# ShangtongZhang/DeepRL

Hardware: AMD Instinct MI355X
Metric: gradient-updates/sec (higher is better)
Workload: dtype f32; 1 GPU; DQN Breakout 84x84x4 uint8, NatureConvBody, batch 32, 1000000-frame HBM replay ring, centered RMSprop, clip 5 (BASELINE configs[1]); global_batch=32, parallelism=replicas x1, actor_in_step=True, async_actor=True, kernel_variant=530248191

## Files before the change

### deeprl_amd/csrc/actor_env.h

```cpp
#pragma once
#include "common.h"
#include <stddef.h>

constexpr int kMaxEnvSteps = 8;
constexpr size_t kPrmHeadBytes = offsetof(dra_dqn_step_params, idx);
constexpr int kAringSlots = 64;
constexpr size_t kAprmStride = 512;
static_assert(kPrmHeadBytes <= kAprmStride && kPrmHeadBytes % 4 == 0, "parameter ring entry");

__host__ __device__ __forceinline__ uint64_t mix64(uint64_t z) {
  z = (z ^ (z >> 30)) * 0xBF58476D1CE4E5B9ull;
  z = (z ^ (z >> 27)) * 0x94D049BB133111EBull;
  return z ^ (z >> 31);
}

__device__ __forceinline__ uint64_t synth_frame_word(uint64_t seed, int64_t counter, int64_t action, int w) {
  (void)action;
  return mix64(seed * 0x9E3779B97F4A7C15ull + (uint64_t)counter * 882ull + (uint64_t)w);
}
__device__ __forceinline__ double synth_reward(uint64_t seed, int64_t counter) {
  const uint64_t hh = mix64((seed + 1) * 0x9E3779B97F4A7C15ull + (uint64_t)counter);
  const uint32_t u = (uint32_t)(hh >> 32) % 10u;
  return (u == 0) ? -1.0 : ((u == 9) ? 1.0 : 0.0);
}
// ... 94 lines not shown
int dra_actor_c3fc4(const float* y2_planes, const float* w3, const float* b3, const float* w4, const float* b4, float* y3_planes,
                    float* h4, unsigned* flags, int* timeout_flag, void* stream);

typedef unsigned long long ll_t;

struct ActorPersistArgs {
  const float *w1, *b1, *w2, *b2, *w3, *b3, *w4, *b4, *wh, *bh;
  uint8_t* frames; uint8_t* actions; double* rewards; int32_t* masks;
  int64_t ring_cap;
  const uint8_t* aring; unsigned* seq;
  uint8_t* pend_frame; double* pend_reward; int32_t* pend_mask;
  float* q_out;
  float* h4_plain;
  ll_t *y1, *y2p, *y3p, *h4;
  int* abort_word;
  uint64_t seed;
  double coef;
  int done_period, n_actions, n_env;
  int* timeout_flag;
  const int* w4_valid;
  const unsigned long long* fs_count;
  const unsigned long long* fs_need;
  unsigned long long* fs_done_host;
};

constexpr size_t kPersistY1 = 32 * 400, kPersistY2 = 2 * 64 * 81, kPersistY3 = 2 * 64 * 49, kPersistH4 = 2 * 512;
constexpr size_t kPersistLLWords = kPersistY1 + kPersistY2 + kPersistY3 + kPersistH4;
constexpr int kPersistWgs = 32;
int dra_actor_persist(const ActorPersistArgs* a, void* stream);

constexpr int kChainPad = 32;
constexpr int kFwdChainCounters = 2 * DRA_MAX_Z * 32 * kChainPad;
void dra_conv_chain_attach_announce(unsigned long long* count);
void dra_conv_chain_attach_zero(unsigned* word);
int dra_conv_fwd_chain(const void* frames, const int64_t* idx, int64_t* idx_copy, const int64_t* idx_tagged,
                       const unsigned long long* update_seq, const int64_t* newest_off, int nz, const float* const* w1,
                       const float* const* b1, float* const* y1, const float* const* w2, const float* const* b2, float* const* y2,
                       const float* const* w3, const float* const* b3, float* const* y3, int batch, double u8_coef,
                       unsigned* done_counters, const unsigned* epoch, int* timeout_flag, const DraFc4Rider* rider,
                       unsigned* rider_count, int* rider_pending, int* rider_valid, void* stream);

void dra_conv_fwd_chain_level(unsigned epoch, unsigned* image, unsigned* arrivals);

int dra_bwd_chain_counters(void);
struct DraBwdChainFc {
  const float *dq, *h4, *dh4, *x3, *w4;
  float *dwh, *dbh, *dw4, *db4;
  int n_actions, in_features;
  double* sq_partials;
  int* n_sq_partials;
  const int64_t* head_action;
  int head_group;
};
int dra_conv_bwd_chain(const float* dy3, const float* y2, const float* wt3, float* dw3, float* db3, int64_t stride3, float* dy2,
                       const float* y1, const float* wt2, float* dw2, float* db2, int64_t stride2, float* dy1, const void* frames,
                       const int64_t* idx, float* dw1, float* db1, int64_t stride1, int batch, double u8_coef, int act,
                       const dra_fold_seg* fold3, const dra_fold_seg* fold2, float* grad, double* partials3, int* n_partials3,
                       double* partials2, int* n_partials2, double* reset_slots, int n_reset, unsigned* counters,
                       const unsigned* epoch, int* timeout_flag, const DraBwdChainFc* fc, void* stream);
int dra_bwd_chain_level(int batch, int fc_in_features, unsigned epoch, unsigned* image, unsigned* arrivals);
```

### deeprl_amd/csrc/fused.hip

```cpp
#include "oneshot_lin.h"
#include "dgrad_scatter.h"
#include "actor_env.h"
#include "per_chain2.h"
#include <stdlib.h>
#include <type_traits>

static int g_tuning = 511 | 4096 | 8192 | 16384 | 32768 | 131072 | 524288 | 1048576 | 8388608 | 16777216 | 33554432 | 67108864 | 134217728 | 268435456;

DRA_API int dra_set_tuning(int mask) {
  if (mask < 0) return DRA_EINVAL;
  g_tuning = mask;
  return DRA_OK;
}
DRA_API int dra_get_tuning(int* mask) {
  if (!mask) return DRA_EINVAL;
  static bool env_read = false;
  if (!env_read) {
    env_read = true;
    const char* e = getenv("DRA_TUNING");
    if (e && atoi(e) >= 0) g_tuning = atoi(e);
  }
  *mask = g_tuning;
  return DRA_OK;
}
// ... 251 lines not shown
static FoldRole make_fold_role(const dra_fold_seg* fold, float* grad, double* partials, double* reset_slots, int n_reset) {
  FoldRole f;
  f.grad = grad; f.slabs = fold->slabs; f.begin4 = fold->begin >> 2; f.count4 = fold->count >> 2;
  f.stride4 = fold->slab_stride >> 2; f.n_slabs = fold->n_slabs; f.partials = partials;
  f.reset_slots = reset_slots; f.n_reset = reset_slots ? n_reset : 0;
  return f;
}
static bool fold_ok(const dra_fold_seg* fold, const float* grad, const double* partials) {
  return fold && grad && partials && fold->slabs && fold->n_slabs >= 1 && fold->n_slabs <= FoldRole::NG * FoldRole::SPT &&
         fold->count >= 4 && !(fold->begin & 3) &&
         !(fold->count & 3) && !(fold->slab_stride & 3) && !((((uintptr_t)fold->slabs) | ((uintptr_t)grad)) & 15);
}

int dra_conv_bwd_fused_fold(int layer, const float* dy, const void* x, const float* wt, const float* xact, float* dw, float* db,
                            int64_t slab_stride, float* dx, int batch, int act, int variant, const dra_fold_seg* fold,
                            float* grad, double* fold_partials, int* n_fold_partials, double* reset_slots, int n_reset,
                            void* stream) {
  if (!dy || !x || !wt || !dx || !dw || !db || batch < 1 || !n_fold_partials || !fold_ok(fold, grad, fold_partials)) return DRA_EINVAL;
  if (!(variant & DRA_VAR_ONESHOT_WGRAD) || !(variant & DRA_VAR_ONESHOT_DGRAD)) return DRA_EINVAL;
  hipStream_t st = dra_stream(stream);
  const FoldRole f = make_fold_role(fold, grad, fold_partials, reset_slots, n_reset);
  *n_fold_partials = f.blocks();
  if (layer == 2)
    return conv_bwd_fused_t<G2, WG2l, WG2l, FoldRole>(dy, x, wt, xact, dw, db, slab_stride, 1, dx, batch, act, variant, st, f, f.blocks());
  if (layer == 3)
    return conv_bwd_fused_t<G3, WG3l, WG3l, FoldRole>(dy, x, wt, xact, dw, db, slab_stride, 1, dx, batch, act, variant, st, f, f.blocks());
  return DRA_EINVAL;
}

int dra_conv1_wgrad_fold(const float* dy, const void* x, const int64_t* idx, float* dw_slabs, float* db_slabs, int64_t slab_stride,
                         int batch, double u8_coef, int variant, const dra_fold_seg* fold, float* grad, double* fold_partials,
                         int* n_fold_partials, double* reset_slots, int n_reset, const PerChain2Args* chain, void* stream) {
  if (!dy || !x || !dw_slabs || !db_slabs || batch < 1 || !(variant & DRA_VAR_ONESHOT_WGRAD) || !n_fold_partials ||
      !fold_ok(fold, grad, fold_partials))
    return DRA_EINVAL;
  const FoldRole f = make_fold_role(fold, grad, fold_partials, reset_slots, n_reset);
  *n_fold_partials = f.blocks();
  if (chain) {
    if (chain->nb > 256) return DRA_EINVAL;
    ChainRole<2> cr;
    cr.a = *chain;
    auto rw = make_wgrad_one<WG1u>(dy, x, dw_slabs, db_slabs, slab_stride, batch, u8_coef);
    rw.sample_idx = idx;
    return launch_multi(rw, rw.blocks(), f, f.blocks(), cr, 1, dra_stream(stream));
  }
  NoRole none;
  auto rw = make_wgrad_one<WG1u>(dy, x, dw_slabs, db_slabs, slab_stride, batch, u8_coef);
  rw.sample_idx = idx;
  return launch_multi(rw, rw.blocks(), f, f.blocks(), none, 0, dra_stream(stream));
}

static bool fc_wgrad_one(int batch) { return batch <= 32; }
constexpr int kFcWgradNI = 8;
struct BwdChainN { int fd, fw, fh, d3, w3, d2, w2, w1, f3, f2; };
using BD3 = ConvDgradLin<G3, 1>;
using BD2 = ConvDgradLin<G2, 2>;
using FCD = LinDgradOne<512>;
using FCW = LinWgradOne<8>;
template <bool FC>
__global__ void __launch_bounds__(256) __attribute__((amdgpu_waves_per_eu(1, 2)))
bwd_chain_kernel(const FCD fd, const FCW fw, const HeadWgradRole fh, const BD3 d3, const WG3l w3, const BD2 d2, const WG2l w2,
                 const WG1u w1, const FoldRole f3, const FoldRole f2, const BwdChainN n) {
  extern __shared__ __attribute__((aligned(16))) float dyn_lds[];
  int b = blockIdx.x, first = 0;
  if constexpr (FC) {
    if (b < n.fd) { fd.run_<true>(b, dyn_lds); return; }
    b -= n.fd; first += n.fd;
    if (b < n.fw) { fw.run(b, dyn_lds, first); return; }
    b -= n.fw; first += n.fw;
    if (b < n.fh) { fh.run(b, dyn_lds, first); return; }
    b -= n.fh; first += n.fh;
  }
  if (b < n.d3) { d3.run_<FC, true>(b, dyn_lds, first); return; }
  b -= n.d3; first += n.d3;
  if (b < n.w3) { w3.run_<FC, true>(b, dyn_lds, first); return; }
  b -= n.w3; first += n.w3;
  if (b < n.d2) { d2.run_<true, true>(b, dyn_lds, first); return; }
  b -= n.d2; first += n.d2;
  if (b < n.w2) { w2.run_<true, true>(b, dyn_lds, first); return; }
  b -= n.w2; first += n.w2;
  if (b < n.w1) { w1.run_<true>(b, dyn_lds, first); return; }
  b -= n.w1;
  if (b < n.f3) { f3.run_<true>(b, dyn_lds); return; }
  b -= n.f3;
  f2.run_<true>(b, dyn_lds);
}

constexpr int kBwdChainCounters = (2 * 32 + 3) * kChainLine;
int dra_bwd_chain_counters(void) { return kBwdChainCounters; }
constexpr int kBwdChainA = 0, kBwdChainB = 32 * kChainLine, kBwdChainW3 = 64 * kChainLine, kBwdChainW2 = 65 * kChainLine,
              kBwdChainF = 66 * kChainLine;
struct BwdChainArrivals { unsigned d3, d2, w3, w2, fd; };
static int fc_dgrad_tiles(int in_features) { return (in_features + 31) / 32; }
static BwdChainArrivals bwd_chain_arrivals(int batch, int fc_in_features) {
  WG3l w3; w3.B = batch;
  WG2l w2; w2.B = batch;
  BwdChainArrivals n;
  n.d3 = BD3::WGS_PER_SAMPLE; n.d2 = BD2::WGS_PER_SAMPLE; n.w3 = (unsigned)w3.blocks(); n.w2 = (unsigned)w2.blocks();
  n.fd = fc_in_features > 0 ? (unsigned)(fc_dgrad_tiles(fc_in_features) * ((batch + 31) / 32)) : 0u;
  return n;
}
int dra_bwd_chain_level(int batch, int fc_in_features, unsigned epoch, unsigned* image, unsigned* arrivals) {
  if (batch < 1 || batch > 32 || !arrivals) return DRA_EINVAL;
  const BwdChainArrivals n = bwd_chain_arrivals(batch, fc_in_features);
  arrivals[0] = n.d3; arrivals[1] = n.d2; arrivals[2] = n.w3; arrivals[3] = n.w2; arrivals[4] = n.fd;
  if (!image) return DRA_OK;
  for (int i = 0; i < 32 * kChainLine; ++i) { image[kBwdChainA + i] = epoch * n.d3; image[kBwdChainB + i] = epoch * n.d2; }
  for (int i = 0; i < kChainLine; ++i) {
    image[kBwdChainW3 + i] = epoch * n.w3; image[kBwdChainW2 + i] = epoch * n.w2; image[kBwdChainF + i] = epoch * n.fd;
  }
  return DRA_OK;
}

int dra_conv_bwd_chain(const float* dy3, const float* y2, const float* wt3, float* dw3, float* db3, int64_t stride3, float* dy2,
                       const float* y1, const float* wt2, float* dw2, float* db2, int64_t stride2, float* dy1, const void* frames,
                       const int64_t* idx, float* dw1, float* db1, int64_t stride1, int batch, double u8_coef, int act,
                       const dra_fold_seg* fold3, const dra_fold_seg* fold2, float* grad, double* partials3, int* n_partials3,
                       double* partials2, int* n_partials2, double* reset_slots, int n_reset, unsigned* counters,
                       const unsigned* epoch, int* timeout_flag, const DraBwdChainFc* fc, void* stream) {
  if (!dy3 || !y2 || !wt3 || !dw3 || !db3 || !dy2 || !y1 || !wt2 || !dw2 || !db2 || !dy1 || !frames || !dw1 || !db1 || batch < 1 ||
      batch > 32 || !n_partials3 || !n_partials2 || !fold_ok(fold3, grad, partials3) || !fold_ok(fold2, grad, partials2) || !counters ||
      !epoch || !timeout_flag)
    return DRA_EINVAL;
  if (kWideLd4 && ((int64_t)fold3->n_slabs * fold3->slab_stride * 4 >= (1ll << 31) || (int64_t)fold2->n_slabs * fold2->slab_stride * 4 >= (1ll << 31)))
    return DRA_EINVAL;
  BD3 d3 = make_dgrad_one<G3, 1>(dy3, wt3, y2, dy2, batch, act);
  WG3l w3 = make_wgrad_one<WG3l>(dy3, y2, dw3, db3, stride3, batch, 1.0);
  BD2 d2 = make_dgrad_one<G2, 2>(dy2, wt2, y1, dy1, batch, act);
  WG2l w2 = make_wgrad_one<WG2l>(dy2, y1, dw2, db2, stride2, batch, 1.0);
  WG1u w1 = make_wgrad_one<WG1u>(dy1, frames, dw1, db1, stride1, batch, u8_coef);
  w1.sample_idx = idx;
  FoldRole f3 = make_fold_role(fold3, grad, partials3, nullptr, 0);
  FoldRole f2 = make_fold_role(fold2, grad, partials2, reset_slots, n_reset);
  BwdChainN n;
  n.fd = n.fw = n.fh = 0;
  n.d3 = d3.blocks(); n.w3 = w3.blocks(); n.d2 = d2.blocks(); n.w2 = w2.blocks(); n.w1 = w1.blocks(); n.f3 = f3.blocks(); n.f2 = f2.blocks();
  *n_partials3 = n.f3; *n_partials2 = n.f2;
  unsigned *cA = counters + kBwdChainA, *cB = counters + kBwdChainB, *cW3 = counters + kBwdChainW3, *cW2 = counters + kBwdChainW2,
           *cF = counters + kBwdChainF;
  const BwdChainArrivals na = bwd_chain_arrivals(batch, fc ? fc->in_features : 0);
  if (n.w3 != (int)na.w3 || n.w2 != (int)na.w2 || n.d3 != (int)na.d3 * batch || n.d2 != (int)na.d2 * batch) return DRA_EINVAL;
  ChainHook base;
  base.epoch = epoch; base.epoch_bias = 0; base.timeout_flag = timeout_flag;
  FCD fd = {};
  FCW fw = {};
  HeadWgradRole fh;
  fh.dq = nullptr; fh.h4 = nullptr; fh.dwh = nullptr; fh.dbh = nullptr; fh.B = 0; fh.A = 0;
  if (fc) {
    if (!fc->dq || !fc->h4 || !fc->dh4 || !fc->x3 || !fc->w4 || !fc->dwh || !fc->dbh || !fc->dw4 || !fc->db4 || fc->n_actions < 1 ||
        fc->in_features != G3::OC * G3::P || !fc->sq_partials || !fc->n_sq_partials || !fc_wgrad_one(batch))
      return DRA_EINVAL;
    fd.dy = fc->dh4; fd.w = fc->w4; fd.xact = fc->x3; fd.dx = const_cast<float*>(dy3); fd.B = batch; fd.I = fc->in_features; fd.act = act;
    fd.tiles_n = fc_dgrad_tiles(fc->in_features);
    fd.hook = base; fd.hook.done = cF;
    fw.dy = fc->dh4; fw.x = fc->x3; fw.dw = fc->dw4; fw.db = fc->db4; fw.partials = fc->sq_partials; fw.B = batch; fw.O = 512;
    fw.I = fc->in_features; fw.tiles_o = 512 / 32; fw.groups_i = (fd.tiles_n + kFcWgradNI - 1) / kFcWgradNI;
    fh.dq = fc->dq; fh.h4 = fc->h4; fh.dwh = fc->dwh; fh.dbh = fc->dbh; fh.B = batch; fh.A = fc->n_actions;
    if (fc->head_action && fc->head_group > 1 && fc->n_actions % fc->head_group == 0) { fh.action = fc->head_action; fh.group = fc->head_group; }
    n.fd = (int)na.fd; n.fw = fw.blocks(); n.fh = 2 * fc->n_actions;
    fh.partials = fc->sq_partials + n.fw;
    *fc->n_sq_partials = n.fw + 2 * fc->n_actions;
  }
  d3.hook = base; d3.hook.done = cA; d3.hook.done_stride = kChainLine;
  w3.hook = base; w3.hook.done = cW3;
  if (fc) {
    d3.hook.wait = cF; d3.hook.wait_stride = 0; d3.hook.wait_target = na.fd; d3.hook.slow = 1;
    w3.hook.wait = cF; w3.hook.wait_stride = 0; w3.hook.wait_target = na.fd; w3.hook.slow = 1;
  }
  d2.hook = base; d2.hook.wait = cA; d2.hook.wait_stride = kChainLine; d2.hook.wait_target = na.d3;
  d2.hook.done = cB; d2.hook.done_stride = kChainLine;
  w2.hook = base; w2.hook.wait = cA; w2.hook.wait_stride = kChainLine; w2.hook.wait_target = na.d3; w2.hook.done = cW2;
  w1.hook = base; w1.hook.wait = cB; w1.hook.wait_stride = kChainLine; w1.hook.wait_target = na.d2;
  f3.hook = base; f3.hook.wait = cW3; f3.hook.wait_target = na.w3; f3.hook.slow = 1;
  f2.hook = base; f2.hook.wait = cW2; f2.hook.wait_target = na.w2; f2.hook.slow = 1;
  constexpr int fa = BD3::LDS_FLOATS > WG3l::LDS_FLOATS ? BD3::LDS_FLOATS : WG3l::LDS_FLOATS;
  constexpr int fb = BD2::LDS_FLOATS > WG2l::LDS_FLOATS ? BD2::LDS_FLOATS : WG2l::LDS_FLOATS;
  constexpr int fcl = WG1u::LDS_FLOATS > FoldRole::LDS_FLOATS ? WG1u::LDS_FLOATS : FoldRole::LDS_FLOATS;
  constexpr int fab = fa > fb ? fa : fb, fl = fab > fcl ? fab : fcl;
  constexpr size_t bytes = (size_t)fl * sizeof(float);
  static_assert(bytes <= 64 * 1024, "LDS per workgroup of the chained backward launch");
  const int grid = n.fd + n.fw + n.fh + n.d3 + n.w3 + n.d2 + n.w2 + n.w1 + n.f3 + n.f2;
  if (fc) {
    constexpr size_t bytes_fc = (size_t)(FCD::LDS_FLOATS > fl ? FCD::LDS_FLOATS : fl) * sizeof(float);
    static_assert(bytes_fc <= 80 * 1024, "two workgroups of the chained backward launch per CU");
    static DraLdsAttr lds_attr;
    if (bytes_fc > 64 * 1024)
      if (int rc = dra_grant_lds(lds_attr, reinterpret_cast<const void*>(&bwd_chain_kernel<true>), bytes_fc)) return rc;
    hipLaunchKernelGGL(bwd_chain_kernel<true>, dim3(grid), dim3(256), bytes_fc, dra_stream(stream), fd, fw, fh, d3, w3, d2, w2, w1, f3, f2, n);
  } else {
    hipLaunchKernelGGL(bwd_chain_kernel<false>, dim3(grid), dim3(256), bytes, dra_stream(stream), fd, fw, fh, d3, w3, d2, w2, w1, f3, f2, n);
  }
  DRA_LAUNCH_CHECK();
  return DRA_OK;
}

int dra_fc_bwd_fused_sq_partials(int batch, int n_actions, int in_features) {
  const int tiles_i = (in_features + 31) / 32;
  const int nw = fc_wgrad_one(batch) ? (512 / 32) * ((tiles_i + kFcWgradNI - 1) / kFcWgradNI) : (512 / 64) * ((in_features + 1 + 63) / 64);
  return nw + 2 * n_actions;
}

int dra_fc_bwd_fused_sq(const float* dq, const float* h4, const float* dh4, const float* x3, const float* w4, float* dwh,
                        float* dbh, float* dw4, float* db4, float* dx3, int batch, int n_actions, int in_features, int act,
                        int variant, double* sq_partials, int* n_sq_partials, const int64_t* head_action, int head_group,
                        void* stream) {
  if (!dq || !h4 || !dh4 || !x3 || !w4 || !dwh || !dbh || !dw4 || !db4 || !dx3 || batch < 1 || n_actions < 1 ||
      in_features < 1 || !sq_partials || !n_sq_partials || !(variant & DRA_VAR_ONESHOT_DGRAD))
    return DRA_EINVAL;
  hipStream_t st = dra_stream(stream);
  constexpr int O = 512;
  LinDgradOne<O> rd;
  rd.dy = dh4; rd.w = w4; rd.xact = x3; rd.dx = dx3; rd.B = batch; rd.I = in_features; rd.act = act;
  rd.tiles_n = (in_features + 31) / 32;
  HeadWgradRole rh;
  rh.dq = dq; rh.h4 = h4; rh.dwh = dwh; rh.dbh = dbh; rh.B = batch; rh.A = n_actions;
  if (head_action && head_group > 1 && n_actions % head_group == 0) { rh.action = head_action; rh.group = head_group; }
  if (fc_wgrad_one(batch)) {
    constexpr int NI = kFcWgradNI;
    LinWgradOne<NI> rl;
    rl.dy = dh4; rl.x = x3; rl.dw = dw4; rl.db = db4; rl.partials = sq_partials; rl.B = batch; rl.O = O; rl.I = in_features;
    rl.tiles_o = O / 32; rl.groups_i = (rd.tiles_n + NI - 1) / NI;
    const int nw = rl.blocks();
    rh.partials = sq_partials + nw;
    *n_sq_partials = nw + 2 * n_actions;
    return launch_multi(rd, rd.tiles_n * ((batch + 31) / 32), rl, nw, rh, 2 * n_actions, st);
  }
  LinWgradSq<64, 64, 32> pw;
  pw.M = O; pw.N = in_features + 1; pw.K = batch; pw.I = in_features; pw.dy = dh4; pw.x = x3; pw.dw = dw4; pw.db = db4;
  pw.partials = sq_partials;
  auto rw = make_igemm_role(pw, 1);
  const int nw = igemm_blocks(rw, 1);
  rh.partials = sq_partials + nw;
  *n_sq_partials = nw + 2 * n_actions;
  return launch_multi(rd, rd.tiles_n * ((batch + 31) / 32), rw, nw, rh, 2 * n_actions, st);
}

DRA_API int dra_fc_bwd_fused(const float* dq, const float* h4, const float* dh4, const float* x3, const float* w4,
                             float* dwh, float* dbh, float* dw4, float* db4, float* dx3, int batch, int n_actions,
                             int in_features, int act, int variant, void* stream) {
  if (!dq || !h4 || !dh4 || !x3 || !w4 || !dwh || !dbh || !dw4 || !db4 || !dx3 || batch < 1 || n_actions < 1 ||
      in_features < 1)
// ... 100 lines not shown
```

### deeprl_amd/csrc/learner.hip

```cpp
#include "oneshot_lin.h"
#include "actor_env.h"
#include "per_chain2.h"
#include "cached_graph.h"
#include <new>
#include <stddef.h>
#include <stdlib.h>
#include <string.h>
#include <vector>

enum { K_GATHER, K_CONV1_F, K_CONV2_F, K_CONV3_F, K_FC4_F, K_HEAD, K_HEAD_BW, K_FC4_BW, K_FC4_BX, K_CONV3_BW, K_CONV3_BX,
       K_CONV2_BW, K_CONV2_BX, K_CONV1_BW, K_NORM, K_STEP, K_COUNT };

static const char* kKernelNames[K_COUNT] = {
  "gather", "conv1_fwd", "conv2_fwd", "conv3_fwd", "fc4_fwd", "head_loss", "head_bwd_w", "fc4_bwd_w", "fc4_bwd_x",
  "conv3_bwd_w", "conv3_bwd_x", "conv2_bwd_w", "conv2_bwd_x", "conv1_bwd_w", "grad_norm", "rmsprop_step"};

enum { P_W1, P_B1, P_W2, P_B2, P_W3, P_B3, P_W4, P_B4, P_WH, P_BH, P_COUNT };

constexpr int kFc4Split = 8;
constexpr int kFc4SplitWide = 28;
constexpr int kFc4SplitMid = 14;
static int fc4_ks(const struct dra_dqn_learner* l);
constexpr int kAprmSlots = 16;

// ... 43 lines not shown
  int ag_prev_par;
  hipEvent_t* tr_ev;
  int tr_cap, tr_n;
  double host_wait_s, host_call_s;
  int64_t host_calls;
  struct { CachedGraph g; const float* params; int n_env; } g_actor[5];
  float* pa[4];
  hipEvent_t pa_reader[4];
  int pa_cur;
  bool pa_valid;
  float* ah4;
  uint8_t* qs_stage;
  float* q_stage;
  unsigned* q_seq_dev;
  unsigned q_seq_host;
  CachedGraph g_q;
  uint8_t* aprm_ring;
  unsigned* aprm_seq_dev;
  unsigned* fc4_ticket;
  uint64_t aprm_seq;
  uint8_t* aring_dev;
  uint8_t* aring_stage;
  unsigned* aring_seq;
  uint8_t* pend_frame;
  double* pend_reward;
  int32_t* pend_mask;
  uint64_t aring_pushed, aring_issued;
  bool aring_primed;
  CachedGraph g_aring[4];
  int g_aring_nenv[4];
  hipEvent_t aprm_ev[16];
  bool aprm_used[16];
  hipStream_t side;
  hipEvent_t ev_fork, ev_join[4];
  hipEvent_t ev_actor_done, ev_gather_done, ev_step_done;
  hipEvent_t last_done;
  bool actor_pending;
  int step_per;
  float step_beta;
  int64_t* idx_pin[4];
  CachedGraph g_rd[4], g_rd_per[4], g_rd_per_b[4];
  hipEvent_t ev_upd[4];
  bool upd_used[4];
  int rd_slot;
  int keep_minibatch;
  struct { hipEvent_t ev; int n; int64_t slots[8]; } arec[8];
  int arec_count;
  hipEvent_t actor_last = nullptr;
  hipEvent_t ev[K_COUNT + 1];
  bool profiling;
  int only_kernel;
  int only_chain;
  unsigned* hchain_dev;
  bool defer;
  float* defer_dev;
  bool defer_host;
  int defer_q;
  int rider_q;
  int64_t defer_begin, defer_count;
  hipEvent_t ev_flush;
  int* timeout_flag;
  int64_t* idx_tag_pin[4];
  int64_t* idx_tag_dev;
  unsigned long long* rd_seq_dev;
  uint64_t rd_issued;
  float* sp_stage;
  hipEvent_t sp_ev[8];
  bool sp_used[8];
  int sp_k;
  int64_t* ui_stage;
  hipEvent_t ui_ev[8];
  bool ui_used[8];
  int ui_k;
  CachedGraph g_qa[2];
  hipEvent_t ev_hq[2];
  int64_t hq_updates;
  bool hq_seeded;
  dra_sumtree* per_tree;
  double* per_stat;
  dra_per_chain2_io* per2_io[4];
  void* per2_dev;
  int64_t* per2_idx;
  const uint32_t* per2_words;
  int split_q;
  hipEvent_t split_opt_prev;
  bool split_seed, split_open;
  bool per2_active;
  bool per2_ride;
  bool per2_split;
  PerChain2Args per2_args;
  unsigned* fchain_dev;
  bool fchain;
  unsigned* bchain_dev;
  bool bchain;
  unsigned long long* all_dev;
  int actor_cus;
  unsigned* aflags;
  bool fs, fs_on;
  unsigned long long* fs_count;
  uint64_t fs_issued;
  unsigned long long* fs_host;
  bool fs_graph[4];
  bool fs_agraph[4];
  bool fs_persist_taken;
  bool fs_capturing;
  uint64_t fs_need_next;
// ... 88 lines not shown
       (cfg->head_kind == DRA_HEAD_CATEGORICAL && !(cfg->v_max > cfg->v_min))))
    return DRA_EINVAL;
  dra_dqn_learner* l = new (std::nothrow) dra_dqn_learner();
  if (!l) return DRA_ENOMEM;
  memset(l, 0, sizeof(*l));
  l->c = *cfg; l->ring = ring; l->p = params; l->pt = target; l->g = grad; l->s1 = state1; l->s2 = state2;
  l->rd_slot = -1;
  l->only_kernel = -1;
  if (cfg->head_kind == DRA_HEAD_QUANTILE) l->c.double_q = 0;
  const int B = cfg->batch, A = cfg->n_actions;
  const int nz = l->c.double_q ? 3 : 2;
  const int NO = cfg->head_kind == DRA_HEAD_VANILLA ? A : A * cfg->n_atoms;
  l->n_out = NO;
  int rc = 0;
  for (int g = 0; g < 2; ++g) {
    rc |= (int)hipMalloc(&l->state_[g], (size_t)B * 4 * 7056);
    rc |= (int)hipMalloc(&l->next_state_[g], (size_t)B * 4 * 7056);
    rc |= (int)hipMalloc(&l->action_[g], (size_t)B * 8);
    rc |= alloc_f(&l->reward_[g], B); rc |= alloc_f(&l->mask_[g], B);
  }
  rc |= (int)hipMalloc(&l->act_state, (size_t)4 * 7056);
  rc |= (int)hipMalloc(&l->idx, (size_t)B * 8);
  for (int z = 0; z < nz; ++z) {
    rc |= alloc_f(&l->y1[z], (int64_t)B * 32 * 400); rc |= alloc_f(&l->y2[z], (int64_t)B * 64 * 81);
    rc |= alloc_f(&l->y3[z], (int64_t)B * 64 * 49); rc |= alloc_f(&l->q[z], (int64_t)B * NO);
  }
  rc |= alloc_f(&l->h4, (int64_t)3 * B * 512);
  rc |= (int)hipMalloc(&l->opt_step, sizeof(int64_t));
  if (!rc) rc |= (int)hipMemset(l->opt_step, 0, sizeof(int64_t));
  if (cfg->head_kind != DRA_HEAD_VANILLA) {
    const int N = cfg->n_atoms;
    rc |= alloc_f(&l->atoms, N); rc |= alloc_f(&l->qr_ws, (int64_t)B * N); rc |= alloc_f(&l->alog, NO);
    if (!rc) {
      float host_atoms[1024];
      const double step = ((double)cfg->v_max - (double)cfg->v_min) / (double)(N - 1);
      for (int i = 0; i < N; ++i) host_atoms[i] = (float)((double)cfg->v_min + (double)i * step);
      host_atoms[N - 1] = cfg->v_max;
      rc |= (int)hipMemcpy(l->atoms, host_atoms, (size_t)N * sizeof(float), hipMemcpyHostToDevice);
    }
  }
  rc |= alloc_f(&l->ay1, 32 * 400); rc |= alloc_f(&l->ay2, 64 * 81); rc |= alloc_f(&l->ay3, 64 * 49);
  rc |= alloc_f(&l->aq, A);
  rc |= alloc_f(&l->ay2p, 2 * 64 * 81); rc |= alloc_f(&l->ay3p, 2 * 64 * 49);
  rc |= alloc_f(&l->dq, (int64_t)B * NO); rc |= alloc_f(&l->dh4, (int64_t)B * 512);
  rc |= alloc_f(&l->dy3, (int64_t)B * 64 * 49); rc |= alloc_f(&l->dy2, (int64_t)B * 64 * 81);
  rc |= alloc_f(&l->dy1, (int64_t)B * 32 * 400);
  rc |= alloc_f(&l->delta, (cfg->head_kind == DRA_HEAD_QUANTILE && cfg->n_atoms > B) ? cfg->n_atoms : B);
  rc |= alloc_f(&l->prio, B); rc |= alloc_f(&l->weights, B);
  rc |= alloc_f(&l->samp_prob, B + 1);
  l->slab_stride = cfg->conv_end;
  rc |= alloc_f(&l->slabs, (int64_t)cfg->ksplit * l->slab_stride);
  if (cfg->variant >= 0) l->variant = cfg->variant;
  else rc |= dra_get_tuning(&l->variant);
  if ((l->variant & DRA_VAR_RING_DIRECT) &&
      (!(l->variant & DRA_VAR_ONESHOT_WGRAD) || !(l->variant & DRA_VAR_GATHER_ON_UPDATE) || !(l->variant & DRA_VAR_PINNED_IDX)))
    l->variant &= ~DRA_VAR_RING_DIRECT;
  if (cfg->head_kind != DRA_HEAD_VANILLA) {
    l->variant |= DRA_VAR_ACTOR_V2;
    l->variant &= ~(DRA_VAR_ACTOR_V3 | DRA_VAR_ACTOR_FUSED_HEAD | DRA_VAR_GATHER_IN_GRAPH);
  }
  if (l->variant & DRA_VAR_ONESHOT_WGRAD) {
    const int wi[3] = {P_W1, P_W2, P_W3};
    const int64_t seg_end[3] = {cfg->offset[P_W2], cfg->offset[P_W3], cfg->conv_end};
    for (int k = 0; k < 3; ++k) {
      l->lstride[k] = seg_end[k] - cfg->offset[wi[k]];
      rc |= dra_conv_wgrad_slabs(k + 1, B, cfg->ksplit, l->variant, &l->lnslabs[k]);
      if (rc) break;
      rc |= alloc_f(&l->lslabs[k], (int64_t)l->lnslabs[k] * l->lstride[k]);
      if (!rc) rc |= (int)hipMemset(l->lslabs[k], 0, (size_t)l->lnslabs[k] * l->lstride[k] * sizeof(float));
    }
  }
  l->n_partials = 2 * dra_norm_partials();
  if ((l->variant & DRA_VAR_LATE_FOLD) && (l->variant & DRA_VAR_ONESHOT_WGRAD) && (l->variant & DRA_VAR_ONESHOT_DGRAD) &&
      (l->variant & DRA_VAR_FUSED_BWD) && !rc && cfg->offset[P_W1] == 0 && l->lnslabs[1] <= 32 && l->lnslabs[2] <= 32) {
    dra_fold_seg s0;
    memset(&s0, 0, sizeof(s0));
    s0.begin = 0; s0.count = l->lstride[0]; s0.slabs = l->lslabs[0]; s0.slab_stride = l->lstride[0]; s0.n_slabs = l->lnslabs[0];
    if (dra_clip_step_late_blocks(&s0, &l->late_nfold) == DRA_OK) {
      const int64_t np = dra_fc_bwd_fused_sq_partials(cfg->batch, NO, 3136) + (l->lstride[2] / 4 + 63) / 64 + (l->lstride[1] / 4 + 63) / 64 + l->late_nfold;
      l->late = np <= dra_norm_partials_max();
    }
  }
  rc |= alloc_f(&l->ah4, 512);
  l->rider_q = -1;
  l->defer_begin = cfg->offset[P_W4];
  l->defer_count = cfg->offset[P_B4] - cfg->offset[P_W4];
  {
    const int need = DRA_VAR_DEFER_FC4 | DRA_VAR_RING_DIRECT | DRA_VAR_GATHER_ON_UPDATE | DRA_VAR_ACTOR_PARAMS | DRA_VAR_ACTOR_RING |
                     DRA_VAR_ACTOR_FUSED_CONV1 | DRA_VAR_ACTOR_MEGA | DRA_VAR_ONESHOT_FWD;
    l->defer = (l->variant & need) == need && l->late && cfg->head_kind == DRA_HEAD_VANILLA && cfg->optimizer == DRA_OPT_RMSPROP &&
               !cfg->double_q && cfg->batch > 16 && cfg->batch < 128 &&
               (l->defer_begin & 3) == 0 && (l->defer_count & 3) == 0 && l->defer_count == (int64_t)512 * 3136 &&
               l->defer_begin >= l->lstride[0];
  }
  l->fchain = (l->variant & DRA_VAR_FWD_CHAIN) && (l->variant & DRA_VAR_RING_DIRECT) && cfg->head_kind == DRA_HEAD_VANILLA &&
              !cfg->double_q && cfg->batch > 16 && cfg->batch <= 32;
  l->bchain = (l->variant & DRA_VAR_BWD_CHAIN) && (l->variant & DRA_VAR_RING_DIRECT) && l->late && cfg->head_kind == DRA_HEAD_VANILLA &&
              !cfg->double_q && cfg->batch > 16 && cfg->batch <= 32;
  rc |= (int)hipMalloc(&l->bchain_dev, (size_t)dra_bwd_chain_counters() * sizeof(unsigned));
  if (!rc) rc |= (int)hipMemset(l->bchain_dev, 0, (size_t)dra_bwd_chain_counters() * sizeof(unsigned));
  rc |= (int)hipMalloc(&l->defer_dev, 8 * sizeof(float));
  if (!rc) {
    const int init[8] = {0, 0, 1, 1, 1, 1, 0, 0};
    rc |= (int)hipMemcpy(l->defer_dev, init, sizeof(init), hipMemcpyHostToDevice);
  }
  {
    const int need = DRA_VAR_FLAG_SYNC | DRA_VAR_RING_DIRECT | DRA_VAR_GATHER_ON_UPDATE | DRA_VAR_PIPE_GATHER | DRA_VAR_ACTOR_PARAMS |
                     DRA_VAR_ACTOR_RING | DRA_VAR_ACTOR_FUSED_CONV1 | DRA_VAR_ACTOR_MEGA | DRA_VAR_ACTOR_PERSIST;
    l->fs = (l->variant & need) == need && l->fchain && cfg->head_kind == DRA_HEAD_VANILLA &&
            !(l->variant & (DRA_VAR_GATHER_IN_GRAPH | DRA_VAR_ACTOR_V3));
  }
  rc |= (int)hipMalloc(&l->fs_count, 256);
  if (!rc) rc |= (int)hipMemset(l->fs_count, 0, 256);
  rc |= (int)hipHostMalloc(&l->fs_host, (size_t)(8 + kAringSlots) * sizeof(unsigned long long), hipHostMallocDefault);
  if (!rc) memset(l->fs_host, 0, (size_t)(8 + kAringSlots) * sizeof(unsigned long long));
  rc |= (int)hipEventCreateWithFlags(&l->ev_fs, hipEventDisableTiming);
  rc |= (int)hipMalloc(&l->aflags, (size_t)kMaxEnvSteps * 4 * sizeof(unsigned));
  rc |= (int)hipMalloc(&l->hchain_dev, 256);
  if (!rc) rc |= (int)hipMemset(l->hchain_dev, 0, 256);
  rc |= (int)hipMalloc(&l->fchain_dev, (size_t)(kFwdChainCounters + 2) * sizeof(unsigned));
  if (!rc) rc |= (int)hipMemset(l->fchain_dev, 0, (size_t)(kFwdChainCounters + 2) * sizeof(unsigned));
  l->ah = false;
  if ((l->variant & DRA_VAR_TARGET_AHEAD) && l->fs && (l->variant & DRA_VAR_LANE_EAGER) && l->bchain && !cfg->double_q && B <= 32 &&
      (l->variant & DRA_VAR_ONESHOT_FWD)) {
    for (int k = 0; k < 2; ++k) {
      rc |= alloc_f(&l->ah_y1[k], (int64_t)B * 32 * 400); rc |= alloc_f(&l->ah_y2[k], (int64_t)B * 64 * 81);
      rc |= alloc_f(&l->ah_y3[k], (int64_t)B * 64 * 49); rc |= alloc_f(&l->ah_slabs[k], (int64_t)kFc4SplitWide * B * 512);
      rc |= (int)hipMalloc(&l->ah_chain[k], (size_t)(kFwdChainCounters + 2) * sizeof(unsigned));
      if (!rc) rc |= (int)hipMemset(l->ah_chain[k], 0, (size_t)(kFwdChainCounters + 2) * sizeof(unsigned));
    }
    for (int k = 0; k < 8; ++k) rc |= (int)hipHostMalloc(&l->ah_idx_pin[k], 1024 * sizeof(int64_t), hipHostMallocDefault);
    rc |= (int)hipMalloc(&l->ah_idx_copy, 1024 * sizeof(int64_t));
    rc |= (int)hipMalloc(&l->ah_done, 256);
    if (!rc) rc |= (int)hipMemset(l->ah_done, 0, 256);
  }
  {
    const size_t words = kPersistLLWords + 1;
    rc |= (int)hipMalloc(&l->all_dev, words * sizeof(unsigned long long));
    if (!rc) rc |= (int)hipMemset(l->all_dev, 0, words * sizeof(unsigned long long));
  }
  if (!rc) rc |= (int)hipMemset(l->aflags, 0, (size_t)kMaxEnvSteps * 4 * sizeof(unsigned));
  if (l->variant & DRA_VAR_ACTOR_PARAMS) { rc |= alloc_f(&l->pa[0], cfg->n_params); rc |= alloc_f(&l->pa[1], cfg->n_params); }
  if ((l->variant & DRA_VAR_ACTOR_PARAMS) && (l->variant & DRA_VAR_GATHER_ON_UPDATE)) {
    rc |= alloc_f(&l->pa[2], cfg->n_params); rc |= alloc_f(&l->pa[3], cfg->n_params);
  }
  if (l->variant & DRA_VAR_ACTOR_V3) {
    rc |= (int)hipHostMalloc(&l->aprm_ring, kAprmSlots * kAprmStride, hipHostMallocDefault);
    rc |= (int)hipMalloc(&l->aprm_seq_dev, sizeof(unsigned));
    rc |= (int)hipMalloc(&l->fc4_ticket, sizeof(unsigned));
    if (!rc) rc |= (int)hipMemset(l->aprm_seq_dev, 0, sizeof(unsigned));
    if (!rc) rc |= (int)hipMemset(l->fc4_ticket, 0, sizeof(unsigned));
    for (int k = 0; k < kAprmSlots; ++k) rc |= (int)hipEventCreateWithFlags(&l->aprm_ev[k], hipEventDisableTiming);
  }
  if (l->variant & DRA_VAR_ACTOR_RING) {
    rc |= (int)hipMalloc(&l->aring_dev, kAringSlots * kAprmStride);
    rc |= (int)hipHostMalloc(&l->aring_stage, kAringSlots * kAprmStride, hipHostMallocDefault);
    rc |= (int)hipMalloc(&l->aring_seq, sizeof(unsigned));
    rc |= (int)hipMalloc(&l->pend_frame, 7056);
    rc |= (int)hipMalloc(&l->pend_reward, sizeof(double));
    rc |= (int)hipMalloc(&l->pend_mask, sizeof(int32_t));
    if (!rc) rc |= (int)hipMemset(l->aring_seq, 0, sizeof(unsigned));
    if (!rc) rc |= (int)hipMemset(l->aring_dev, 0, kAringSlots * kAprmStride);
  }
  rc |= alloc_f(&l->fc4_slabs, (int64_t)3 * kFc4SplitWide * B * 512);
  rc |= alloc_f(&l->afc4_slabs, (int64_t)kFc4Split * 512);
  l->lin_ws_floats = (int64_t)3 * 32 * B * 512;
  rc |= alloc_f(&l->lin_ws, l->lin_ws_floats);
  rc |= (int)hipMalloc(&l->partials, (size_t)dra_norm_partials_max() * sizeof(double));
  rc |= alloc_f(&l->loss, 1); rc |= alloc_f(&l->norm, 1);
  if (l->variant & DRA_VAR_IDX_PREFETCH) {
    if (!(l->variant & DRA_VAR_RING_DIRECT) || cfg->ring_capacity >= (1ll << 40)) l->variant &= ~DRA_VAR_IDX_PREFETCH;
  }
// ... 31 lines not shown
  rc |= (int)hipMemset(l->slabs, 0, (size_t)cfg->ksplit * l->slab_stride * sizeof(float));
  rc |= (int)hipMemset(l->partials, 0, (size_t)dra_norm_partials_max() * sizeof(double));
  rc |= (int)hipMemset(l->prm_dev, 0, sizeof(dra_dqn_step_params));
  for (int k = 0; k <= K_COUNT; ++k) rc |= (int)hipEventCreate(&l->ev[k]);
  for (int k = 0; k < 8; ++k) rc |= (int)hipEventCreateWithFlags(&l->stage_ev[k], hipEventDisableTiming);
  for (int k = 0; k < 2; ++k) rc |= (int)hipEventCreateWithFlags(&l->ev_hq[k], hipEventDisableTiming);
  rc |= (int)hipStreamCreateWithFlags(&l->side, hipStreamNonBlocking);
  rc |= (int)hipEventCreateWithFlags(&l->ev_fork, hipEventDisableTiming);
  for (int k = 0; k < 4; ++k) rc |= (int)hipEventCreateWithFlags(&l->ev_join[k], hipEventDisableTiming);
  rc |= (int)hipEventCreateWithFlags(&l->ev_actor_done, hipEventDisableTiming);
  rc |= (int)hipEventCreateWithFlags(&l->ev_loss, hipEventDisableTiming);
  rc |= (int)hipEventCreateWithFlags(&l->ev_gather_done, hipEventDisableTiming);
  rc |= (int)hipEventCreateWithFlags(&l->ev_step_done, hipEventDisableTiming);
  rc |= (int)hipEventCreateWithFlags(&l->ev_flush, hipEventDisableTiming);
  for (int g = 0; g < 2; ++g) {
    rc |= (int)hipEventCreateWithFlags(&l->ev_mb_ready[g], hipEventDisableTiming);
    rc |= (int)hipEventCreateWithFlags(&l->ev_mb_free[g], hipEventDisableTiming);
  }
  if (rc) { delete l; return rc; }
  *out = l;
  return DRA_OK;
}

DRA_API int dra_dqn_learner_destroy(dra_dqn_learner* l) {
  if (!l) return DRA_OK;
  (void)hipDeviceSynchronize();
  l->g_update.reset();
  l->g_update_per.reset();
  l->g_q.reset();
  for (auto& g : l->g_ag) g.reset();
  for (auto& g : l->g_qa) g.reset();
  for (auto& ga : l->g_actor) ga.g.reset();
  for (int k = 0; k < 4; ++k) {
    l->g_pipe[k].reset(); l->g_pipe_per[k].reset(); l->g_pipe_per_b[k].reset();
    l->g_rd[k].reset(); l->g_rd_per[k].reset(); l->g_rd_per_b[k].reset();
    l->g_aring[k].reset();
  }
  if (l->tr_ev) {
    for (int i = 0; i < l->tr_cap * 5; ++i) (void)hipEventDestroy(l->tr_ev[i]);
    delete[] l->tr_ev;
  }
  for (int g = 0; g < 2; ++g) {
    (void)hipEventDestroy(l->ev_mb_ready[g]); (void)hipEventDestroy(l->ev_mb_free[g]);
    void* mb[] = {l->state_[g], l->next_state_[g], l->action_[g], l->reward_[g], l->mask_[g]};
    for (void* b : mb) if (b) (void)hipFree(b);
  }
  for (int k = 0; k < 4; ++k) if (l->pa[k]) (void)hipFree(l->pa[k]);
  if (l->ah4) (void)hipFree(l->ah4);
  if (l->defer_dev) (void)hipFree(l->defer_dev);
  if (l->aflags) (void)hipFree(l->aflags);
  if (l->all_dev) (void)hipFree(l->all_dev);
  if (l->fchain_dev) (void)hipFree(l->fchain_dev);
  if (l->hchain_dev) (void)hipFree(l->hchain_dev);
  for (int k = 0; k < 2; ++k) {
    void* ab[] = {l->ah_y1[k], l->ah_y2[k], l->ah_y3[k], l->ah_slabs[k], l->ah_chain[k]};
    for (void* b : ab) if (b) (void)hipFree(b);
  }
  for (int k = 0; k < 8; ++k) if (l->ah_idx_pin[k]) (void)hipHostFree(l->ah_idx_pin[k]);
  if (l->ah_idx_copy) (void)hipFree(l->ah_idx_copy);
  if (l->ah_done) (void)hipFree(l->ah_done);
  if (l->bchain_dev) (void)hipFree(l->bchain_dev);
  if (l->fs_count) (void)hipFree(l->fs_count);
  if (l->fs_host) (void)hipHostFree(l->fs_host);
  if (l->ev_fs) (void)hipEventDestroy(l->ev_fs);
  if (l->aring_dev) {
    (void)hipFree(l->aring_dev); (void)hipHostFree(l->aring_stage); (void)hipFree(l->aring_seq);
    (void)hipFree(l->pend_frame); (void)hipFree(l->pend_reward); (void)hipFree(l->pend_mask);
  }
  if (l->aprm_ring) {
    (void)hipHostFree(l->aprm_ring); (void)hipFree(l->aprm_seq_dev); (void)hipFree(l->fc4_ticket);
    for (int k = 0; k < kAprmSlots; ++k) (void)hipEventDestroy(l->aprm_ev[k]);
  }
  void* bufs[] = {l->act_state, l->idx, l->h4, l->ay1, l->ay2,
                  l->ay3, l->aq, l->dq, l->dh4, l->dy3, l->dy2, l->dy1, l->delta, l->prio, l->weights, l->samp_prob,
                  l->slabs, l->fc4_slabs, l->afc4_slabs, l->lin_ws, l->partials, l->loss, l->norm, l->prm_dev};
  for (void* b : bufs) if (b) (void)hipFree(b);
  void* hb[] = {l->atoms, l->qr_ws, l->alog, l->opt_step, l->ay2p, l->ay3p};
  for (void* b : hb) if (b) (void)hipFree(b);
  for (int k = 0; k < 3; ++k) if (l->lslabs[k]) (void)hipFree(l->lslabs[k]);
  for (int z = 0; z < 3; ++z) {
    if (l->y1[z]) (void)hipFree(l->y1[z]);
    if (l->y2[z]) (void)hipFree(l->y2[z]);
    if (l->y3[z]) (void)hipFree(l->y3[z]);
    if (l->q[z]) (void)hipFree(l->q[z]);
  }
  (void)hipHostFree(l->prm_stage);
  (void)hipHostFree(l->idx_stage);
  for (int k = 0; k < 4; ++k) {
    if (l->idx_pin[k]) (void)hipHostFree(l->idx_pin[k]);
    (void)hipEventDestroy(l->ev_upd[k]);
  }
  for (int k = 0; k < 4; ++k) if (l->idx_tag_pin[k]) (void)hipHostFree(l->idx_tag_pin[k]);
  if (l->idx_tag_dev) (void)hipFree(l->idx_tag_dev);
  if (l->per2_dev) (void)hipFree(l->per2_dev);
  if (l->per2_idx) (void)hipFree(l->per2_idx);
  if (l->rd_seq_dev) (void)hipFree(l->rd_seq_dev);
  if (l->sp_stage) (void)hipHostFree(l->sp_stage);
  for (int k = 0; k < 8; ++k) if (l->sp_ev[k]) (void)hipEventDestroy(l->sp_ev[k]);
  if (l->ui_stage) (void)hipHostFree(l->ui_stage);
  for (int k = 0; k < 8; ++k) if (l->ui_ev[k]) (void)hipEventDestroy(l->ui_ev[k]);
  if (l->timeout_flag) (void)hipHostFree(l->timeout_flag);
  if (l->qs_stage) (void)hipHostFree(l->qs_stage);
  if (l->q_stage) (void)hipHostFree(l->q_stage);
  if (l->q_seq_dev) (void)hipFree(l->q_seq_dev);
  for (int k = 0; k < 2; ++k) {
    if (l->ev_hq[k]) (void)hipEventDestroy(l->ev_hq[k]);
// ... 374 lines not shown

template <int KS>
__global__ void __launch_bounds__(256)
head_fused_kernel(const float* __restrict__ slabs, int nz, int B, int A, const float* __restrict__ b4_on,
                  const float* __restrict__ b4_tg, const float* __restrict__ wh_on, const float* __restrict__ wh_tg,
                  const float* __restrict__ bh_on, const float* __restrict__ bh_tg, const int64_t* __restrict__ action,
                  const float* __restrict__ reward, const float* __restrict__ mask, float gamma_n, int double_q,
                  float* __restrict__ h4_out, float* __restrict__ q_on, float* __restrict__ q_tg, float* __restrict__ q_on2,
                  float* __restrict__ delta, float* __restrict__ dq, float* __restrict__ dh4, int64_t* __restrict__ opt_step,
                  const RingScalars rs, const float* __restrict__ per_w, const float* __restrict__ pf_w4) {
  __shared__ float s_h[3][512];
  __shared__ float s_q[3][64];
  const int b = blockIdx.x, tid = threadIdx.x;
  if (b >= B) {
    const int pcol = (b - B) * 32;
    float4 v[16];
#pragma unroll
    for (int qq = 0; qq < 16; ++qq) {
      const int e = tid + 256 * qq, row = e >> 3, c4 = e & 7;
      v[qq] = *reinterpret_cast<const float4*>(pf_w4 + (int64_t)row * 3136 + pcol + 4 * c4);
    }
#pragma unroll
    for (int qq = 0; qq < 16; ++qq) asm volatile("" :: "v"(v[qq].x), "v"(v[qq].y), "v"(v[qq].z), "v"(v[qq].w));
    return;
  }
  head_fused_body<KS, false>(slabs, nz, B, A, b4_on, b4_tg, wh_on, wh_tg, bh_on, bh_tg, action, reward, mask, gamma_n, double_q, h4_out, q_on, q_tg, q_on2, delta, dq, dh4, opt_step, rs, per_w, b, s_h, s_q, nullptr);
}

struct HeadArgs {
  const float* slabs; int nz, B, A;
  const float *b4_on, *b4_tg, *wh_on, *wh_tg, *bh_on, *bh_tg;
  const int64_t* action; const float *reward, *mask; float gamma_n; int double_q;
  float *h4_out, *q_on, *q_tg, *q_on2, *delta, *dq, *dh4; int64_t* opt_step;
  RingScalars rs; const float* per_w; unsigned* done;
};
template <int KS>
__global__ void __launch_bounds__(256) __attribute__((amdgpu_waves_per_eu(1, 2)))
head_fc_bwd_kernel(const HeadArgs ha, const LinDgradOne<512> rd, const LinWgradOne<8> rl, const HeadWgradRole rh, const int nd, const int nw) {
  extern __shared__ __attribute__((aligned(16))) float dyn_lds[];
  int b = blockIdx.x;
  if (b < ha.B) {
    float (*s_h)[512] = reinterpret_cast<float (*)[512]>(dyn_lds);
    float (*s_q)[64] = reinterpret_cast<float (*)[64]>(dyn_lds + 3 * 512);
    head_fused_body<KS, true>(ha.slabs, ha.nz, ha.B, ha.A, ha.b4_on, ha.b4_tg, ha.wh_on, ha.wh_tg, ha.bh_on, ha.bh_tg, ha.action, ha.reward,
                              ha.mask, ha.gamma_n, ha.double_q, ha.h4_out, ha.q_on, ha.q_tg, ha.q_on2, ha.delta, ha.dq, ha.dh4, ha.opt_step,
                              ha.rs, ha.per_w, b, s_h, s_q, ha.done);
    return;
  }
  b -= ha.B;
  if (b < nd) { rd.run_<false, true>(b, dyn_lds); return; }
  b -= nd;
  if (b < nw) { rl.run_<true>(b, dyn_lds); return; }
  rh.run_<true>(b - nw, dyn_lds);
}

__global__ void __launch_bounds__(64)
head_wgrad_kernel(const float* __restrict__ dq, const float* __restrict__ h4, int B, int A, float* __restrict__ dwh,
                  float* __restrict__ dbh) {
  const int a = blockIdx.x, k = blockIdx.y * 64 + threadIdx.x;
  float acc = 0.f, accb = 0.f;
  int b = 0;
  for (; b + 8 <= B; b += 8) {
    float d[8], h[8];
#pragma unroll
    for (int i = 0; i < 8; ++i) { d[i] = dq[(int64_t)(b + i) * A + a]; h[i] = h4[(int64_t)(b + i) * 512 + k]; }
#pragma unroll
    for (int i = 0; i < 8; ++i) { acc += d[i] * h[i]; accb += d[i]; }
  }
  for (; b < B; ++b) {
    const float d = dq[(int64_t)b * A + a];
    acc += d * h4[(int64_t)b * 512 + k];
    accb += d;
  }
  dwh[a * 512 + k] = acc;
  if (k == 0) dbh[a] = accb;
}

#define STEP(kid, expr)                                                        \
  do {                                                                         \
    if (l->only_kernel >= 0 && l->only_kernel != (kid)) break;                 \
    if (l->profiling) DRA_HIP(hipEventRecord(l->ev[kid], st));                 \
    int _rc = (expr);                                                          \
    if (_rc != DRA_OK) return _rc;                                             \
  } while (0)

static int launch_gather(dra_dqn_learner* l, hipStream_t st, const int64_t* idx = nullptr) {
  l->last_gb = l->gb;
  return dra_ring_gather(l->ring, idx ? idx : l->idx, l->c.batch, l->state_[l->gb], l->next_state_[l->gb], l->action_[l->gb], nullptr, nullptr,
                         l->reward_[l->gb], l->mask_[l->gb], (void*)st);
}

struct BodyFlags {
  dra_dqn_learner* const l;
  BodyFlags(dra_dqn_learner* l_, int gb, int rd_slot = -1, int rider_q = -1, bool fs_capturing = false, bool per2_active = false,
            int only_kernel = -1, int only_chain = 0) : l(l_) {
    l->gb = gb; l->rd_slot = rd_slot; l->rider_q = rider_q; l->fs_capturing = fs_capturing; l->per2_active = per2_active;
    l->only_kernel = only_kernel; l->only_chain = only_chain;
  }
  BodyFlags(const BodyFlags&) = delete;
  BodyFlags& operator=(const BodyFlags&) = delete;
  ~BodyFlags() {
    l->gb = 0; l->rd_slot = -1; l->rider_q = -1; l->fs_capturing = false;
    l->per2_active = l->per2_ride = l->per2_split = false;
    l->only_kernel = -1; l->only_chain = 0;
  }
};
// ... 180 lines not shown
  if (fc4_ks(l) == kFc4SplitWide)
    hipLaunchKernelGGL(fc4_reduce_kernel<kFc4SplitWide>, dim3(B, nz), dim3(256), 0, st, (const float*)l->fc4_slabs, B, P + o[P_B4],
                       T + o[P_B4], l->h4, l->opt_step, rs);
  else if (fc4_ks(l) == kFc4SplitMid)
    hipLaunchKernelGGL(fc4_reduce_kernel<kFc4SplitMid>, dim3(B, nz), dim3(256), 0, st, (const float*)l->fc4_slabs, B, P + o[P_B4],
                       T + o[P_B4], l->h4, l->opt_step, rs);
  else
    hipLaunchKernelGGL(fc4_reduce_kernel<kFc4Split>, dim3(B, nz), dim3(256), 0, st, (const float*)l->fc4_slabs, B, P + o[P_B4],
                       T + o[P_B4], l->h4, l->opt_step, rs);
  DRA_LAUNCH_CHECK();
  int rc = DRA_OK;
  {
    const float* hx[3] = {l->h4, l->h4 + (int64_t)B * 512, l->h4 + (int64_t)2 * B * 512};
    const float* hw[3] = {P + o[P_WH], T + o[P_WH], P + o[P_WH]};
    const float* hb[3] = {P + o[P_BH], T + o[P_BH], P + o[P_BH]};
    if ((rc = dra_head_fwd_one(nz, hx, hw, hb, l->q, B, NO, s))) return rc;
  }
  if (c.head_kind == DRA_HEAD_CATEGORICAL) {
    const float* weights = nullptr;
    if (per) {
      if (!l->per2_active &&
          (rc = dra_per_weights(nullptr, l->samp_prob, B, beta, c.replay_eps, c.replay_alpha, nullptr, l->weights, s))) return rc;
      weights = l->weights;
    }
    rc = dra_c51_loss(l->q[0], l->q[1], c.double_q ? l->q[2] : nullptr, l->action_[l->gb], 1, l->reward_[l->gb], l->mask_[l->gb],
                      B, A, N, c.gamma_n, c.v_min, c.v_max, l->atoms, l->delta, l->dq, weights, s);
    if (rc) return rc;
    if (per && !l->per2_active &&
        (rc = dra_per_weights(l->delta, l->samp_prob, B, beta, c.replay_eps, c.replay_alpha, l->prio, nullptr, s))) return rc;
  } else {
    if (per) return DRA_EINVAL;
    rc = dra_qr_loss(l->q[0], l->q[1], l->action_[l->gb], 1, l->reward_[l->gb], l->mask_[l->gb], B, A, N, c.gamma_n, l->qr_ws,
                     l->delta, l->loss, l->dq, s);
    if (rc) return rc;
  }
  hipLaunchKernelGGL(dist_head_dgrad_kernel, dim3(B, 4), dim3(256), 0, st, (const float*)l->dq, P + o[P_WH], (const float*)l->h4,
                     (const int64_t*)l->action_[l->gb], N, NO, l->dh4);
  DRA_LAUNCH_CHECK();
  return DRA_OK;
}

static int run_body(dra_dqn_learner* l, hipStream_t st, int per, float beta, int fork, int part = 0) {
  const dra_dqn_config& c = l->c;
  l->captured = true;
  const int B = c.batch, A = c.n_actions;
  const int nz = c.double_q ? 3 : 2;
  void* s = (void*)st;
  const float* P = l->p;
  const float* T = l->pt;
  const int64_t* o = c.offset;
  const bool rd = l->rd_slot >= 0;
  const bool bchain = l->bchain && rd && !l->profiling && l->only_kernel < 0 && part == 0 && !per && !(l->per2_active && l->per2_ride);
  bool head_chain = false;
  void *ring_frames = nullptr, *ring_actions = nullptr, *ring_rewards = nullptr, *ring_masks = nullptr;
  int ring_h = 4, ring_n = 1;
  double ring_discount = 1.0;
  if (rd) {
    int rc0 = dra_ring_pointers(l->ring, &ring_frames, &ring_actions, &ring_rewards, &ring_masks);
    if (!rc0) rc0 = dra_ring_shape(l->ring, &ring_h, &ring_n);
    if (!rc0) rc0 = dra_ring_discount(l->ring, &ring_discount);
    if (rc0) return rc0;
    if (ring_h != 4) return DRA_EINVAL;
  }
  if (part != 2 && l->only_chain != 2) {
  const void* x1[3] = {l->state_[l->gb], l->next_state_[l->gb], l->next_state_[l->gb]};
  const float* w1[3] = {P + o[P_W1], T + o[P_W1], P + o[P_W1]};
  const float* b1[3] = {P + o[P_B1], T + o[P_B1], P + o[P_B1]};
  bool chain = false;
  if (rd) {
    const int64_t off[3] = {0, ring_n, ring_n};
    const bool dev_idx = per && l->per2_dev;
    const bool pf = (l->variant & DRA_VAR_IDX_PREFETCH) && !dev_idx;
    chain = l->fchain && !l->profiling && l->only_kernel < 0 && nz == 2;
    if (!chain && l->rider_q >= 0 && l->only_kernel < 0) {
      const DraFc4Rider r = fc4_rider(l, l->pa[l->rider_q]);
      const int nb = fc4_rider_blocks(r.count4);
      dra_conv_attach_rider(&r, 0, (nb * kRiderConv1Pct) / 100, nullptr, nullptr);
    }
    if (chain) {
      const float* w2c[3] = {P + o[P_W2], T + o[P_W2], P + o[P_W2]};
      const float* b2c[3] = {P + o[P_B2], T + o[P_B2], P + o[P_B2]};
      const float* w3c[3] = {P + o[P_W3], T + o[P_W3], P + o[P_W3]};
      const float* b3c[3] = {P + o[P_B3], T + o[P_B3], P + o[P_B3]};
      const bool riding = l->rider_q >= 0;
      DraFc4Rider rdr;
      if (riding) rdr = fc4_rider(l, l->pa[l->rider_q]);
      if (l->fs_capturing) dra_conv_chain_attach_announce(l->fs_count);
      if ((l->variant & DRA_VAR_HEAD_CHAIN) && l->hchain_dev) dra_conv_chain_attach_zero(l->hchain_dev);
      int rcc = dra_conv_fwd_chain(ring_frames, dev_idx ? l->per2_idx + (size_t)l->rd_slot * 1024 : l->idx_pin[l->rd_slot], l->idx,
                                   pf ? l->idx_tag_dev + (size_t)l->rd_slot * 1024 : nullptr, pf ? l->rd_seq_dev : nullptr, off,
                                   l->ah_mode ? 1 : nz,
                                   w1, b1, l->y1, w2c, b2c, l->y2, w3c, b3c, l->y3, B, c.u8_coef, l->fchain_dev,
                                   l->fchain_dev + kFwdChainCounters, l->timeout_flag, riding ? &rdr : nullptr,
                                   l->fchain_dev + kFwdChainCounters + 1, defer_pending_word(l),
                                   defer_valid_word(l, l->rider_q >= 0 ? l->rider_q : 0), s);
      if (rcc) return rcc;
      if (l->only_chain == 1) return DRA_OK;
      if (l->ah_mode == 2)
        if (int rct = ah_target_launches(l, st, (int)(l->step_no & 1), l->idx_pin[l->rd_slot], false, 0)) return rct;
    } else
    STEP(K_CONV1_F, dra_conv1_fwd_koc_ringbatch(ring_frames, dev_idx ? l->per2_idx + (size_t)l->rd_slot * 1024 : l->idx_pin[l->rd_slot], l->idx,
                                                pf ? l->idx_tag_dev + (size_t)l->rd_slot * 1024 : nullptr, pf ? l->rd_seq_dev : nullptr,
                                                off, nz, w1, b1, l->y1, B, c.u8_coef, DRA_ACT_RELU, s));
  } else {
    STEP(K_CONV1_F, dra_conv_fwd_koc(1, nz, x1, w1, b1, l->y1, B, 1, c.u8_coef, DRA_ACT_RELU, s));
  }
  const void* x2[3] = {l->y1[0], l->y1[1], l->y1[2]};
  const float* w2[3] = {P + o[P_W2], T + o[P_W2], P + o[P_W2]};
  const float* b2[3] = {P + o[P_B2], T + o[P_B2], P + o[P_B2]};
  if (!chain && rd && l->rider_q >= 0 && l->only_kernel < 0) {
    const DraFc4Rider r = fc4_rider(l, l->pa[l->rider_q]);
    const int nb = fc4_rider_blocks(r.count4);
    dra_conv_attach_rider(&r, (nb * kRiderConv1Pct) / 100, nb - (nb * kRiderConv1Pct) / 100, nullptr, nullptr);
  }
  if (!chain)
  STEP(K_CONV2_F, dra_conv_fwd_koc(2, nz, x2, w2, b2, l->y2, B, 0, 1.0, DRA_ACT_RELU, s));
  const void* x3[3] = {l->y2[0], l->y2[1], l->y2[2]};
  const float* w3[3] = {P + o[P_W3], T + o[P_W3], P + o[P_W3]};
  const float* b3[3] = {P + o[P_B3], T + o[P_B3], P + o[P_B3]};
  const float* x4[3] = {l->y3[0], l->y3[1], l->y3[2]};
  const float* w4[3] = {P + o[P_W4], T + o[P_W4], P + o[P_W4]};
  const int ks4 = fc4_ks(l);
  if (!chain && rd && l->rider_q >= 0 && l->only_kernel < 0)
    dra_conv_attach_rider(nullptr, 0, 0, defer_pending_word(l), defer_valid_word(l, l->rider_q));
  if (chain) {
  } else if ((l->variant & DRA_VAR_ONESHOT_FWD) && ks4 == kFc4SplitMid && nz == 2 && B <= 32)
    STEP(K_CONV3_F, dra_conv3_fwd_koc_pf(nz, x3, w3, b3, l->y3, B, DRA_ACT_RELU, w4, nz, s));
  else
  STEP(K_CONV3_F, dra_conv_fwd_koc(3, nz, x3, w3, b3, l->y3, B, 0, 1.0, DRA_ACT_RELU, s));
  if (chain && l->ah_mode == 2) x4[1] = l->ah_y3[l->step_no & 1];
  if (l->variant & DRA_VAR_ONESHOT_FWD) STEP(K_FC4_F, dra_linear_fwd_slabs_one((chain && l->ah_mode == 1) ? 1 : nz, x4, w4, B, 3136, 512, ks4, l->fc4_slabs, s));
  else STEP(K_FC4_F, dra_linear_fwd_slabs(nz, x4, w4, B, 3136, 512, kFc4Split, l->fc4_slabs, s));
  if (l->profiling) DRA_HIP(hipEventRecord(l->ev[K_HEAD], st));
  RingScalars rs;
  memset(&rs, 0, sizeof(rs));
  if (rd) {
    rs.idx = l->idx; rs.actions = (const uint8_t*)ring_actions; rs.rewards = (const double*)ring_rewards;
    rs.masks = (const int32_t*)ring_masks; rs.n_step = ring_n; rs.discount = ring_discount;
    rs.out_action = l->action_[l->gb]; rs.out_reward = l->reward_[l->gb]; rs.out_mask = l->mask_[l->gb];
    if ((l->variant & DRA_VAR_IDX_PREFETCH) && l->only_kernel < 0) rs.seq = l->rd_seq_dev;
    if (chain || bchain) rs.chain_epoch = l->fchain_dev + kFwdChainCounters;
    if (chain && l->ah_mode == 1) {
      rs.z1_slabs = l->ah_slabs[l->step_no & 1]; rs.z1_done = l->ah_done; rs.z1_want = l->step_no + 1ull; rs.z1_timeout = l->timeout_flag;
    }
  }
  if (l->only_kernel >= 0 && l->only_kernel != K_HEAD) {
  } else if (c.head_kind != DRA_HEAD_VANILLA) {
    int rc = run_dist_head(l, st, per, beta, rs);
    if (rc) return rc;
  } else {
    const float* per_w = (per && l->per2_active) ? l->weights : nullptr;
    head_chain = (l->variant & DRA_VAR_HEAD_CHAIN) && chain && !per && ks4 == kFc4SplitMid && B <= 32 && nz == 2 && l->late && part == 0 &&
                 !(l->variant & DRA_VAR_BWD_CHAIN_FC) && (l->variant & DRA_VAR_ONESHOT_DGRAD) && l->hchain_dev && !l->profiling;
    const bool pf = (l->variant & DRA_VAR_ONESHOT_DGRAD) && B % 8 == 0 && B <= 32 && dra_xcd_order_enabled();
    const float* pf_w4 = pf ? P + o[P_W4] : nullptr;
    const int hb = B + (pf ? 3136 / 32 : 0);
    l->q_head_chain = head_chain ? 1 : 0; l->q_head_pf = (!head_chain && pf) ? 1 : 0; l->q_head_launches++;
    if (head_chain) {
      HeadArgs ha;
      ha.slabs = l->fc4_slabs; ha.nz = nz; ha.B = B; ha.A = A; ha.b4_on = P + o[P_B4]; ha.b4_tg = T + o[P_B4]; ha.wh_on = P + o[P_WH];
      ha.wh_tg = T + o[P_WH]; ha.bh_on = P + o[P_BH]; ha.bh_tg = T + o[P_BH]; ha.action = (const int64_t*)l->action_[l->gb];
      ha.reward = (const float*)l->reward_[l->gb]; ha.mask = (const float*)l->mask_[l->gb]; ha.gamma_n = c.gamma_n; ha.double_q = c.double_q;
      ha.h4_out = l->h4; ha.q_on = l->q[0]; ha.q_tg = l->q[1]; ha.q_on2 = l->q[2]; ha.delta = l->delta; ha.dq = l->dq; ha.dh4 = l->dh4;
      ha.opt_step = l->opt_step; ha.rs = rs; ha.per_w = nullptr; ha.done = l->hchain_dev;
      ChainHook hk;
      hk.wait = l->hchain_dev; hk.wait_target = (unsigned)B; hk.timeout_flag = l->timeout_flag;
      LinDgradOne<512> rd = {};
      rd.dy = l->dh4; rd.w = P + o[P_W4]; rd.xact = l->y3[0]; rd.dx = l->dy3; rd.B = B; rd.I = 3136; rd.act = DRA_ACT_RELU; rd.tiles_n = 3136 / 32;
      rd.hook = hk;
      LinWgradOne<8> rl = {};
      float* Gh = l->g;
      rl.dy = l->dh4; rl.x = l->y3[0]; rl.dw = Gh + o[P_W4]; rl.db = Gh + o[P_B4]; rl.partials = l->partials; rl.B = B; rl.O = 512; rl.I = 3136;
      rl.tiles_o = 512 / 32; rl.groups_i = (rd.tiles_n + 8 - 1) / 8;
      rl.hook = hk;
      HeadWgradRole rh;
      rh.dq = l->dq; rh.h4 = l->h4; rh.dwh = Gh + o[P_WH]; rh.dbh = Gh + o[P_BH]; rh.B = B; rh.A = A;
      const int nd = rd.tiles_n, nw = rl.blocks();
      rh.partials = l->partials + nw;
      rh.hook = hk;
      if (nw + 2 * A != dra_fc_bwd_fused_sq_partials(B, A, 3136)) return DRA_EINVAL;
      constexpr size_t hbytes = (size_t)LinDgradOne<512>::LDS_FLOATS * sizeof(float);
      static DraLdsAttr lds_attr;
      if (int rcl = dra_grant_lds(lds_attr, reinterpret_cast<const void*>(&head_fc_bwd_kernel<kFc4SplitMid>), hbytes)) return rcl;
      hipLaunchKernelGGL(head_fc_bwd_kernel<kFc4SplitMid>, dim3(B + nd + nw + 2 * A), dim3(256), hbytes, st, ha, rd, rl, rh, nd, nw);
    } else
    if (ks4 == kFc4SplitWide)
      hipLaunchKernelGGL(head_fused_kernel<kFc4SplitWide>, dim3(hb), dim3(256), 0, st, (const float*)l->fc4_slabs, nz, B, A,
                         P + o[P_B4], T + o[P_B4], P + o[P_WH], T + o[P_WH], P + o[P_BH], T + o[P_BH],
                         (const int64_t*)l->action_[l->gb], (const float*)l->reward_[l->gb], (const float*)l->mask_[l->gb], c.gamma_n,
                         c.double_q,
                         l->h4, l->q[0], l->q[1], l->q[2], l->delta, l->dq, l->dh4, l->opt_step, rs, per_w, pf_w4);
    else if (ks4 == kFc4SplitMid)
      hipLaunchKernelGGL(head_fused_kernel<kFc4SplitMid>, dim3(hb), dim3(256), 0, st, (const float*)l->fc4_slabs, nz, B, A,
                         P + o[P_B4], T + o[P_B4], P + o[P_WH], T + o[P_WH], P + o[P_BH], T + o[P_BH],
                         (const int64_t*)l->action_[l->gb], (const float*)l->reward_[l->gb], (const float*)l->mask_[l->gb], c.gamma_n,
                         c.double_q,
                         l->h4, l->q[0], l->q[1], l->q[2], l->delta, l->dq, l->dh4, l->opt_step, rs, per_w, pf_w4);
    else
      hipLaunchKernelGGL(head_fused_kernel<kFc4Split>, dim3(hb), dim3(256), 0, st, (const float*)l->fc4_slabs, nz, B, A,
                         P + o[P_B4], T + o[P_B4], P + o[P_WH], T + o[P_WH], P + o[P_BH], T + o[P_BH],
                         (const int64_t*)l->action_[l->gb], (const float*)l->reward_[l->gb], (const float*)l->mask_[l->gb], c.gamma_n,
                         c.double_q,
                         l->h4, l->q[0], l->q[1], l->q[2], l->delta, l->dq, l->dh4, l->opt_step, rs, per_w, pf_w4);
    DRA_LAUNCH_CHECK();
    if (per && !per_w) {
      int rc = dra_td_loss(l->q[0], l->q[1], c.double_q ? l->q[2] : nullptr, l->action_[l->gb], 1, l->reward_[l->gb],
                           l->mask_[l->gb], B, A, c.gamma_n,
                           l->samp_prob, beta, c.replay_eps, c.replay_alpha, l->loss, l->dq, l->delta, l->prio, l->weights, s);
      if (rc) return rc;
      rc = dra_linear_bwd_x(l->dq, P + o[P_WH], l->h4, l->dh4, B, 512, A, DRA_ACT_RELU, s);
      if (rc) return rc;
    }
  }
  }
  if (part == 1) return DRA_OK;
  const int NO = l->n_out;
  float* G = l->g;
  float* S = l->slabs;
  if (l->variant & (DRA_VAR_FUSED_BWD | DRA_VAR_ONESHOT_WGRAD)) {
    const int var = l->variant;
    const bool own = var & DRA_VAR_ONESHOT_WGRAD;
    float* dw[3]; float* dbs[3]; int64_t stride[3];
    const int wi[3] = {P_W1, P_W2, P_W3}, bi_[3] = {P_B1, P_B2, P_B3};
    for (int k = 0; k < 3; ++k) {
      dw[k] = own ? l->lslabs[k] : S + o[wi[k]];
      dbs[k] = own ? l->lslabs[k] + (o[bi_[k]] - o[wi[k]]) : S + o[bi_[k]];
      stride[k] = own ? l->lstride[k] : l->slab_stride;
    }
    if (l->profiling) { DRA_HIP(hipEventRecord(l->ev[K_HEAD_BW], st)); DRA_HIP(hipEventRecord(l->ev[K_FC4_BW], st)); }
    if (l->late) {
      dra_fold_seg segs[3];
      conv_fold_segs(l, segs);
      const int nfc_expect = dra_fc_bwd_fused_sq_partials(B, NO, 3136), n3_expect = (int)((l->lstride[2] / 4 + 63) / 64), n2_expect = (int)((l->lstride[1] / 4 + 63) / 64);
      const bool fc_in_chain = bchain && (l->variant & DRA_VAR_BWD_CHAIN_FC) && B <= 32 && !head_chain;
      int nfc = (l->only_kernel >= 0 || (l->only_chain == 2 && !fc_in_chain) || head_chain) ? nfc_expect : 0, n3 = l->only_kernel >= 0 ? n3_expect : 0, n2 = l->only_kernel >= 0 ? n2_expect : 0;
      if (l->only_chain != 2 && !fc_in_chain && !head_chain)
      STEP(K_FC4_BX, dra_fc_bwd_fused_sq(l->dq, l->h4, l->dh4, l->y3[0], P + o[P_W4], G + o[P_WH], G + o[P_BH], G + o[P_W4],
                                         G + o[P_B4], l->dy3, B, NO, 3136, DRA_ACT_RELU, var, l->partials, &nfc,
                                         c.head_kind != DRA_HEAD_VANILLA ? l->action_[l->gb] : nullptr, c.n_atoms, s));
      if (l->profiling) DRA_HIP(hipEventRecord(l->ev[K_CONV3_BW], st));
      if (bchain) {
        DraBwdChainFc fcb;
        if (fc_in_chain) {
          fcb.dq = l->dq; fcb.h4 = l->h4; fcb.dh4 = l->dh4; fcb.x3 = l->y3[0]; fcb.w4 = P + o[P_W4]; fcb.dwh = G + o[P_WH];
          fcb.dbh = G + o[P_BH]; fcb.dw4 = G + o[P_W4]; fcb.db4 = G + o[P_B4]; fcb.n_actions = NO; fcb.in_features = 3136;
          fcb.sq_partials = l->partials; fcb.n_sq_partials = &nfc;
          fcb.head_action = c.head_kind != DRA_HEAD_VANILLA ? l->action_[l->gb] : nullptr; fcb.head_group = c.n_atoms;
        }
        int rcb = dra_conv_bwd_chain(l->dy3, l->y2[0], P + o[P_W3], dw[2], dbs[2], stride[2], l->dy2, l->y1[0], P + o[P_W2], dw[1],
                                     dbs[1], stride[1], l->dy1, ring_frames, l->idx, dw[0], dbs[0], stride[0], B, c.u8_coef,
                                     DRA_ACT_RELU, &segs[2], &segs[1], G, l->partials + nfc_expect, &n3,
                                     l->partials + nfc_expect + n3_expect, &n2,
                                     l->partials + nfc_expect + n3_expect + n2_expect, l->late_nfold, l->bchain_dev,
                                     l->fchain_dev + kFwdChainCounters, l->timeout_flag, fc_in_chain ? &fcb : nullptr, s);
        if (rcb) return rcb;
        if (nfc != nfc_expect || n3 != n3_expect || n2 != n2_expect) return DRA_EINVAL;
        l->late_nprior = nfc + n3 + n2;
        return DRA_OK;
      }
      if (l->per2_active && l->per2_ride)
        STEP(K_CONV3_BX, dra_conv3_bwd_fused_chain(l->dy3, l->y2[0], P + o[P_W3], l->y2[0], dw[2], dbs[2], stride[2], l->dy2, B,
                                                   DRA_ACT_RELU, var, &l->per2_args, l->per2_split ? 1 : 0, s));
      else
      STEP(K_CONV3_BX, dra_conv_bwd_fused(3, l->dy3, l->y2[0], P + o[P_W3], l->y2[0], dw[2], dbs[2], stride[2], c.ksplit,
                                          l->dy2, B, 0, 1.0, DRA_ACT_RELU, var, s));
      if (l->profiling) DRA_HIP(hipEventRecord(l->ev[K_CONV2_BW], st));
      STEP(K_CONV2_BX, dra_conv_bwd_fused_fold(2, l->dy2, l->y1[0], P + o[P_W2], l->y1[0], dw[1], dbs[1], stride[1], l->dy1, B,
                                               DRA_ACT_RELU, var, &segs[2], G, l->partials + nfc, &n3, nullptr, 0, s));
      STEP(K_CONV1_BW, dra_conv1_wgrad_fold(l->dy1, rd ? ring_frames : (const void*)l->state_[l->gb], rd ? l->idx : nullptr, dw[0],
                                            dbs[0], stride[0], B, c.u8_coef, var, &segs[1], G, l->partials + nfc + n3, &n2,
                                            l->partials + nfc_expect + n3_expect + n2_expect, l->late_nfold,
                                            (l->per2_active && l->per2_ride && l->per2_split) ? &l->per2_args : nullptr, s));
      if (nfc != nfc_expect || n3 != n3_expect || n2 != n2_expect) return DRA_EINVAL;
      l->late_nprior = nfc + n3 + n2;
      if (l->profiling) { DRA_HIP(hipEventRecord(l->ev[K_NORM], st)); DRA_HIP(hipEventRecord(l->ev[K_STEP], st)); }
      return DRA_OK;
    }
    STEP(K_FC4_BX, dra_fc_bwd_fused(l->dq, l->h4, l->dh4, l->y3[0], P + o[P_W4], G + o[P_WH], G + o[P_BH], G + o[P_W4],
                                    G + o[P_B4], l->dy3, B, NO, 3136, DRA_ACT_RELU, var, s));
    if (l->profiling) DRA_HIP(hipEventRecord(l->ev[K_CONV3_BW], st));
    if (l->per2_active && l->per2_ride)
      STEP(K_CONV3_BX, dra_conv3_bwd_fused_chain(l->dy3, l->y2[0], P + o[P_W3], l->y2[0], dw[2], dbs[2], stride[2], l->dy2, B,
                                                 DRA_ACT_RELU, var, &l->per2_args, 0, s));
    else
    STEP(K_CONV3_BX, dra_conv_bwd_fused(3, l->dy3, l->y2[0], P + o[P_W3], l->y2[0], dw[2], dbs[2], stride[2], c.ksplit,
                                        l->dy2, B, 0, 1.0, DRA_ACT_RELU, var, s));
    if (l->profiling) DRA_HIP(hipEventRecord(l->ev[K_CONV2_BW], st));
    STEP(K_CONV2_BX, dra_conv_bwd_fused(2, l->dy2, l->y1[0], P + o[P_W2], l->y1[0], dw[1], dbs[1], stride[1], c.ksplit,
                                        l->dy1, B, 0, 1.0, DRA_ACT_RELU, var, s));
    if (rd) {
      STEP(K_CONV1_BW, dra_conv1_wgrad_ringbatch(l->dy1, ring_frames, l->idx, dw[0], dbs[0], stride[0], B, c.u8_coef, var, s));
    } else {
      STEP(K_CONV1_BW, dra_conv_bwd_fused(1, l->dy1, l->state_[l->gb], nullptr, nullptr, dw[0], dbs[0], stride[0], c.ksplit, nullptr,
                                          B, 1, c.u8_coef, DRA_ACT_RELU, var, s));
    }
    if (own) {
      dra_fold_seg segs[3];
      conv_fold_segs(l, segs);
      int np_out = 0;
      STEP(K_NORM, dra_grad_sqnorm_segs(G, c.n_params, segs, 3, l->partials, &np_out, s));
      l->n_partials = np_out;
      if (l->profiling) DRA_HIP(hipEventRecord(l->ev[K_STEP], st));
      return DRA_OK;
    }
    const int np = dra_norm_partials();
    STEP(K_NORM, dra_grad_sqnorm(G, c.conv_end, S, c.ksplit, l->slab_stride, l->partials, s));
    if (l->profiling) DRA_HIP(hipEventRecord(l->ev[K_STEP], st));
// ... 248 lines not shown
      for (int r = 0; r < reps && rcb == DRA_OK; ++r) {
        if (pass == 0) rcb = run_body(l, st, 0, 0.f, 0);
        else hipLaunchKernelGGL(empty_probe_kernel, dim3(224), dim3(256), 0, st, (const int*)nullptr);
      }
      return rcb;
    });
    if (rc == DRA_OK) rc = g.launch(st);
    if (rc == DRA_OK) rc = (int)hipStreamSynchronize(st);
    float best = 0.f;
    for (int t = 0; t < 3 && rc == DRA_OK; ++t) {
      float ms = 0.f;
      rc = timed_replay(g, st, l->ev[0], l->ev[1], &ms);
      if (t == 0 || ms < best) best = ms;
    }
    g.reset();
    if (rc != DRA_OK) return rc;
    us[pass] = best * 1e3f / (float)reps;
  }
  out_us[0] = us[0];
  out_us[1] = us[1];
  return DRA_OK;
}

DRA_API int dra_dqn_learner_chain_replay(dra_dqn_learner* l, int which, int reps, float* out_us, void* stream) {
  if (!l || !out_us || reps < 1 || reps > 4096 || which < 0 || which > 1) return DRA_EINVAL;
  if (!(l->variant & DRA_VAR_RING_DIRECT) || !l->late || (which == 0 ? !l->fchain : !l->bchain) || l->c.double_q) return DRA_EINVAL;
  if (int rcl = fs_leave_any(l)) return rcl;
  hipStream_t st = dra_stream(stream);
  if (int rcf = flush_fc4(l, st)) return rcf;
  DRA_HIP(hipStreamSynchronize(st));
  unsigned* epoch = l->fchain_dev + kFwdChainCounters;
  float us[2] = {0.f, 0.f};
  for (int pass = 0; pass < 2; ++pass) {
    CachedGraph g = {};
    int rc = g.capture(st, [&] {
      BodyFlags f(l, 0, 0, -1, false, false, -1, which + 1);
      int rcb = DRA_OK;
      for (int r = 0; r < reps && rcb == DRA_OK; ++r) {
        if (which == 1) hipLaunchKernelGGL(chain_epoch_bump_kernel, dim3(1), dim3(1), 0, st, epoch);
        if (pass == 0) rcb = run_body(l, st, 0, 0.f, 0);
        else hipLaunchKernelGGL(empty_probe_kernel, dim3(224), dim3(256), 0, st, (const int*)nullptr);
        if (which == 0) hipLaunchKernelGGL(chain_epoch_bump_kernel, dim3(1), dim3(1), 0, st, epoch);
      }
      return rcb;
    });
    float best = 0.f;
    for (int t = 0; t < 4 && rc == DRA_OK; ++t) {
      float ms = 0.f;
      rc = timed_replay(g, st, l->ev[0], l->ev[1], &ms);
      if (t == 1 || (t > 1 && ms < best)) best = ms;
    }
    if (rc == DRA_OK) rc = (int)hipMemsetAsync(l->fchain_dev, 0, (size_t)(kFwdChainCounters + 1) * sizeof(unsigned), st);
    if (rc == DRA_OK) rc = (int)hipMemsetAsync(l->bchain_dev, 0, (size_t)dra_bwd_chain_counters() * sizeof(unsigned), st);
    if (rc == DRA_OK) rc = (int)hipStreamSynchronize(st);
    g.reset();
    if (rc != DRA_OK) return rc;
    us[pass] = best * 1e3f / (float)reps;
  }
  out_us[0] = us[0];
  out_us[1] = us[1];
  return *l->timeout_flag ? DRA_ETIMEDOUT : DRA_OK;
}

DRA_API int dra_dqn_learner_chain_set_epoch(dra_dqn_learner* l, uint64_t epoch, int64_t* arrivals, int n_arrivals, void* stream) {
  if (!l || !arrivals || n_arrivals < 8 || epoch > 0xffffffffull) return DRA_EINVAL;
  if (!l->fchain && !l->bchain) return DRA_EINVAL;
  if (int rcl = fs_leave_any(l)) return rcl;
  hipStream_t st = dra_stream(stream);
  if (int rcf = flush_fc4(l, st)) return rcf;
  DRA_HIP(hipStreamSynchronize(st));
  if (l->ah_stream) DRA_HIP(hipStreamSynchronize(l->ah_stream));
  const unsigned e = (unsigned)epoch;
  for (int i = 0; i < 8; ++i) arrivals[i] = 0;
  unsigned fa[2] = {0, 0}, ba[5] = {0, 0, 0, 0, 0};
  std::vector<unsigned> img((size_t)kFwdChainCounters + 1);
  dra_conv_fwd_chain_level(e, img.data(), fa);
  img[kFwdChainCounters] = e;
  DRA_HIP(hipMemcpy(l->fchain_dev, img.data(), img.size() * sizeof(unsigned), hipMemcpyHostToDevice));
  if (l->fchain) { arrivals[0] = fa[0]; arrivals[1] = fa[1]; }
  for (int k = 0; k < 2; ++k)
    if (l->ah_chain[k]) {
      DRA_HIP(hipMemcpy(l->ah_chain[k], img.data(), img.size() * sizeof(unsigned), hipMemcpyHostToDevice));
      arrivals[7] = 1;
    }
  if (l->bchain) {
    const bool fc = (l->variant & DRA_VAR_BWD_CHAIN_FC) != 0;
    std::vector<unsigned> bimg((size_t)dra_bwd_chain_counters());
    if (int rcb = dra_bwd_chain_level(l->c.batch, fc ? 3136 : 0, e, bimg.data(), ba)) return rcb;
    DRA_HIP(hipMemcpy(l->bchain_dev, bimg.data(), bimg.size() * sizeof(unsigned), hipMemcpyHostToDevice));
    for (int i = 0; i < 5; ++i) arrivals[2 + i] = ba[i];
  }
  return DRA_OK;
}

DRA_API int dra_dqn_learner_last_minibatch(dra_dqn_learner* l, void** state, void** next_state, void** action, void** reward,
                                           void** mask) {
  if (!l) return DRA_EINVAL;
  const int g = l->last_gb;
  if (state) *state = l->state_[g];
  if (next_state) *next_state = l->next_state_[g];
  if (action) *action = l->action_[g];
  if (reward) *reward = l->reward_[g];
  if (mask) *mask = l->mask_[g];
  return DRA_OK;
}

DRA_API int dra_dqn_learner_invalidate_actor_copy(dra_dqn_learner* l) {
  if (!l) return DRA_EINVAL;
  l->pa_valid = false;
  l->hq_updates = 0;
  l->hq_seeded = false;
  return DRA_OK;
}

DRA_API int dra_dqn_learner_kernel_name(int k, char* out, int n) {
  if (k < 0 || k >= K_COUNT || !out || n < 1) return DRA_EINVAL;
  strncpy(out, kKernelNames[k], (size_t)n - 1);
  out[n - 1] = 0;
  return DRA_OK;
}

DRA_API int dra_dqn_learner_kernel_count(void) { return K_COUNT; }

DRA_API int dra_dqn_learner_sync_target(dra_dqn_learner* l, void* stream) {
  if (!l) return DRA_EINVAL;
  if (int rcf = flush_fc4(l, dra_stream(stream))) return rcf;
  return dra_copy_f32(l->pt, l->p, l->c.n_params, stream);
}

__global__ void __launch_bounds__(256)
env_stack_kernel(const dra_dqn_step_params* __restrict__ prm, int e, uint8_t* __restrict__ frames,
                 double* __restrict__ rewards, int32_t* __restrict__ masks, int64_t capacity, uint64_t seed,
                 int done_period, uint8_t* __restrict__ stack) {
  const int j = blockIdx.x;
  const int64_t newest = prm->slot[e];
  const int64_t counter = prm->counter[e];
  int64_t slot = newest - 3 + j;
  if (slot < 0) slot += capacity;
  uint64_t* dst = reinterpret_cast<uint64_t*>(stack + (int64_t)j * 7056);
  uint64_t* src = reinterpret_cast<uint64_t*>(frames + slot * 7056);
  if (j == 3 && counter >= 0) {
    const uint64_t base = seed * 0x9E3779B97F4A7C15ull + (uint64_t)counter * 882ull;
    for (int w = threadIdx.x; w < 882; w += blockDim.x) {
// ... 1073 lines not shown
  int rc;
  bool seeded = false;
  const int par = (int)(l->step_no & 1);
  if (prm->n_env > 0) {
    if (l->mb_used[par]) DRA_HIP(hipStreamWaitEvent(sa, l->ev_mb_free[par], 0));
    memcpy(l->prm_stage[k].idx, prm->idx, (size_t)B * sizeof(int64_t));
    DRA_HIP(hipMemcpyAsync(l->prm_dev, &l->prm_stage[k], kPrmHeadBytes + (size_t)B * sizeof(int64_t), hipMemcpyHostToDevice, sa));
    TRACE(0, sa);
    if (l->pa_valid && l->pa_cur != par) l->pa_valid = false;
    if (l->last_done) DRA_HIP(hipStreamWaitEvent(sa, l->last_done, 0));
    if (!l->pa_valid) {
      if ((rc = seed_actor_copy(l, sa, par))) return rc;
      seeded = true;
    }
    if ((rc = ag_graph(l, prm->n_env, par, sa))) return rc;
    DRA_HIP(hipEventRecord(l->ev_mb_ready[par], sa));
    DRA_HIP(hipEventRecord(l->ev_actor_done, sa));
    l->actor_pending = true;
    TRACE(1, sa);
    TRACE(2, sa);
  }
  DRA_HIP(hipEventRecord(l->stage_ev[k], sa));
  if (do_update && l->ag_have_prev) {
    const int q = l->ag_prev_par;
    DRA_HIP(hipStreamWaitEvent(su, l->ev_mb_ready[q], 0));
    if (seeded) DRA_HIP(hipStreamWaitEvent(su, l->ev_join[0], 0));
    TRACE(3, su);
    if ((rc = pipe_graph(l, su, q))) return rc;
    TRACE(4, su);
    if (l->tr_ev && l->tr_n < l->tr_cap) l->tr_n++;
    DRA_HIP(hipEventRecord(l->ev_mb_free[q], su));
    l->last_done = l->ev_mb_free[q];
    l->mb_used[q] = true;
    if (l->pa_valid) l->pa_cur = q;
    l->ag_have_prev = false;
  }
  if (prm->n_env > 0) {
    l->ag_have_prev = true;
    l->ag_prev_par = par;
    l->step_no++;
  }
  return DRA_OK;
}

__global__ void fs_bump_kernel(unsigned long long* count) { __hip_atomic_fetch_add(count, 1ull, __ATOMIC_RELAXED, __HIP_MEMORY_SCOPE_AGENT); }

static int fs_leave(dra_dqn_learner* l, hipStream_t su, hipStream_t sa);
static int fs_leave_any(dra_dqn_learner* l) { return l->fs_on ? fs_leave(l, l->fs_su, l->fs_sa) : DRA_OK; }
static int fs_leave(dra_dqn_learner* l, hipStream_t su, hipStream_t sa) {
  if (!l->fs_on) return DRA_OK;
  l->fs_on = false;
  DRA_HIP(hipStreamSynchronize(su));
  DRA_HIP(hipStreamSynchronize(sa));
  if (l->ah && l->ah_stream) {
    DRA_HIP(hipStreamSynchronize(l->ah_stream));
    l->ah_valid = false;
    l->ah_next_set = false;
    DRA_HIP(hipMemsetAsync(l->fchain_dev, 0, (size_t)(kFwdChainCounters + 1) * sizeof(unsigned), su));
    DRA_HIP(hipMemsetAsync(l->bchain_dev, 0, (size_t)dra_bwd_chain_counters() * sizeof(unsigned), su));
    DRA_HIP(hipStreamSynchronize(su));
  }
  l->last_done = nullptr;
  for (int q = 0; q < 4; ++q) { l->pa_reader[q] = nullptr; l->upd_used[q] = false; l->fs_reader[q] = 0; }
  for (int k = 0; k < 8; ++k) l->stage_used[k] = false;
  l->arec_count = 0;
  l->fs_arec_n = 0;
  DRA_HIP(hipEventRecord(l->ev_fs, sa));
  l->actor_last = l->ev_fs;
  return DRA_OK;
}

static inline uint64_t fs_actor_done(const dra_dqn_learner* l) { return __atomic_load_n(&l->fs_host[0], __ATOMIC_ACQUIRE); }

static inline bool fs_reached(uint64_t done32, uint64_t target) { return (uint32_t)((uint32_t)done32 - (uint32_t)target) < 0x80000000u; }

static int fs_wait_actor(dra_dqn_learner* l, uint64_t target) {
  if (fs_reached(fs_actor_done(l), target)) return DRA_OK;
  HostTimeScope waited(l->host_wait_s);
  for (;;) {
    for (int i = 0; i < 64; ++i) {
      if (fs_reached(fs_actor_done(l), target)) return DRA_OK;
      __builtin_ia32_pause();
    }
    if (*l->timeout_flag) return DRA_ETIMEDOUT;
    if (waited.seconds() > 20.0) return DRA_ETIMEDOUT;
  }
}

static bool fs_eligible(const dra_dqn_learner* l, const dra_dqn_step_params* prm, int do_update, void* stream_actor) {
  if (!l->fs || !stream_actor || !do_update || prm->n_env < 1 || l->step_per || l->keep_minibatch || l->tr_ev) return false;
  const int q = (int)(l->step_no & 3), qr = (q + 3) & 3;
  if (!l->pa_valid || l->pa_cur != qr) return false;
  if (!l->g_rd[q].ready || !l->fs_graph[q]) return false;
  if (!l->g_aring[qr].ready || !l->fs_agraph[qr] || l->g_aring_nenv[qr] != prm->n_env) return false;
  if (!l->aring_primed || l->aring_issued >= l->aring_pushed) return false;
  if (l->defer ? (l->defer_host && l->defer_q != qr) : l->defer_host) return false;
  return true;
}

static int rd_eager(dra_dqn_learner* l, hipStream_t st, int q) {
  l->gb = q & 1;
  l->rd_slot = q;
  l->rider_q = l->defer ? ((q + 3) & 3) : -1;
  l->fs_capturing = true;
  int rc = run_body(l, st, 0, 0.f, 0, 0);
  l->fs_capturing = false;
  l->rider_q = -1;
  if (rc == DRA_OK) rc = launch_optimizer(l, st, l->pa[q], l->defer ? q : -1);
  l->gb = 0;
  l->rd_slot = -1;
  if (rc != DRA_OK) return rc;
  l->fs_issued++;
  if (l->defer) { l->defer_host = true; l->defer_q = q; }
  return DRA_OK;
}

static int step_lane(dra_dqn_learner* l, const dra_dqn_step_params* prm, hipStream_t su, hipStream_t sa) {
  const int B = l->c.batch;
  const int q = (int)(l->step_no & 3), cur = (q + 3) & 3;
  int rc;
  if (!l->fs_on) {
    DRA_HIP(hipStreamSynchronize(su));
    DRA_HIP(hipStreamSynchronize(sa));
    __atomic_store_n(&l->fs_host[0], (unsigned long long)(uint32_t)l->aring_issued, __ATOMIC_RELEASE);
    for (int i = 0; i < 4; ++i) l->fs_reader[i] = 0;
    l->fs_arec_n = 0;
    l->fs_on = true;
    l->fs_stat[1]++;
  }
  const dra_dqn_step_params* ablk =
      reinterpret_cast<const dra_dqn_step_params*>(l->aring_stage + (size_t)(l->aring_issued % kAringSlots) * kAprmStride);
  using clk = std::chrono::steady_clock;
  auto ns = [](clk::time_point a, clk::time_point b) { return (int64_t)std::chrono::duration_cast<std::chrono::nanoseconds>(b - a).count(); };
  const auto tp0 = clk::now();
  if (l->fs_reader[q]) {
    if ((rc = fs_wait_actor(l, l->fs_reader[q]))) return rc;
    l->fs_reader[q] = 0;
  }
  for (int i = l->fs_arec_n - 1; i >= 0; --i) {
    const auto& r = l->fs_arec[i];
    if (fs_reached(fs_actor_done(l), r.done_at)) continue;
    if (gather_reads_slots(l, prm->idx, r.slots, r.n)) {
      {
        HostTimeScope waited(l->host_wait_s);
        DRA_HIP(hipStreamSynchronize(sa));
      }
      l->fs_stat[3]++;
      break;
    }
  }
  const bool hazard = gather_reads_slots(l, prm->idx, ablk->slot, prm->n_env);
  const auto tp1 = clk::now();
  memcpy(l->idx_pin[q], prm->idx, (size_t)B * sizeof(int64_t));
  if (l->variant & DRA_VAR_IDX_PREFETCH) {
    const uint64_t tag = ((l->rd_issued + 1ull) & 0xffffffull) << 40;
    volatile int64_t* dst = l->idx_tag_pin[q];
    for (int b = 0; b < B; ++b) dst[b] = (int64_t)((uint64_t)prm->idx[b] | tag);
    DRA_HIP(hipMemcpyAsync(l->idx_tag_dev + (size_t)q * 1024, l->idx_tag_pin[q], (size_t)B * sizeof(int64_t), hipMemcpyHostToDevice, l->side));
// ... 23 lines not shown
  if (!l->fs_on) return DRA_EINVAL;
  if (hazard) {
    hipLaunchKernelGGL(fs_bump_kernel, dim3(1), dim3(1), 0, su, l->fs_count);
    DRA_LAUNCH_CHECK();
    l->fs_issued++;
    l->fs_stat[2]++;
  }
  l->fs_need_next = l->fs_issued;
  const auto tp3 = clk::now();
  if ((rc = issue_actor_ring(l, prm->n_env, l->pa[cur], cur, sa, true))) return rc;
  const auto tp4 = clk::now();
  l->fs_stat[4] += ns(tp0, tp1); l->fs_stat[5] += ns(tp1, tp2); l->fs_stat[6] += ns(tp2, tp3); l->fs_stat[7] += ns(tp3, tp4);
  l->actor_pending = true;
  const uint64_t done_at = l->aring_issued;
  l->fs_reader[cur] = done_at;
  if (l->fs_arec_n == 4) { for (int i = 1; i < 4; ++i) l->fs_arec[i - 1] = l->fs_arec[i]; l->fs_arec_n = 3; }
  auto& r = l->fs_arec[l->fs_arec_n++];
  r.done_at = done_at; r.n = prm->n_env;
  for (int e = 0; e < prm->n_env && e < 8; ++e) r.slots[e] = ablk->slot[e];
  l->pa_cur = q;
  if (l->ah && l->ah_stream && l->ah_next_set) {
    l->ah_next_set = false;
    bool ok = l->aring_issued < l->aring_pushed;
    for (int i = 0; ok && i < l->fs_arec_n; ++i) {
      const auto& ar = l->fs_arec[i];
      if (!fs_reached(fs_actor_done(l), ar.done_at) && gather_reads_slots(l, l->ah_next_idx, ar.slots, ar.n)) ok = false;
    }
    if (ok) {
      const dra_dqn_step_params* nblk =
          reinterpret_cast<const dra_dqn_step_params*>(l->aring_stage + (size_t)(l->aring_issued % kAringSlots) * kAprmStride);
      if (gather_reads_slots(l, l->ah_next_idx, nblk->slot, nblk->n_env)) ok = false;
    }
    if (ok) {
      const uint64_t nxt = l->step_no + 1;
      int64_t* pin = l->ah_idx_pin[nxt & 7];
      memcpy(pin, l->ah_next_idx, (size_t)B * sizeof(int64_t));
      hipLaunchKernelGGL(ah_gate_kernel, dim3(1), dim3(1), 0, l->ah_stream, (const unsigned long long*)l->fs_count,
                         (unsigned long long)ah_need, l->timeout_flag);
      DRA_LAUNCH_CHECK();
      if ((rc = ah_target_launches(l, l->ah_stream, (int)(nxt & 1), pin, true, nxt + 1ull))) return rc;
      memcpy(l->ah_idx, l->ah_next_idx, (size_t)B * sizeof(int64_t));
      l->ah_for_step = nxt;
      l->ah_valid = true;
    } else {
      l->ah_stat[2]++;
    }
  }
  l->step_no++;
  l->fs_stat[0]++;
  l->fs_stat[8] += ns(tp0, clk::now());
  return DRA_OK;
}

DRA_API int dra_dqn_learner_set_ahead_stream(dra_dqn_learner* l, void* stream) {
  if (!l) return DRA_EINVAL;
  if (int rcl = fs_leave_any(l)) return rcl;
  if (!stream || !l->ah_done) { l->ah = false; l->ah_stream = nullptr; return DRA_OK; }
  l->ah_stream = dra_stream(stream);
  l->ah = true;
  return DRA_OK;
}

DRA_API int dra_dqn_learner_stage_next_indices(dra_dqn_learner* l, const int64_t* idx_next, int n) {
  if (!l || !idx_next || n != l->c.batch || n > 1024) return DRA_EINVAL;
  if (!l->ah) return DRA_OK;
  memcpy(l->ah_next_idx, idx_next, (size_t)n * sizeof(int64_t));
  l->ah_next_set = true;
  return DRA_OK;
}

DRA_API int dra_dqn_learner_ahead_stats(dra_dqn_learner* l, int64_t* out) {
  if (!l || !out) return DRA_EINVAL;
  for (int i = 0; i < 4; ++i) out[i] = l->ah_stat[i];
  out[4] = l->ah ? 1 : 0;
  return DRA_OK;
}

DRA_API int dra_dqn_learner_path_flags(dra_dqn_learner* l, int64_t* out) {
  if (!l || !out) return DRA_EINVAL;
  const int64_t v[12] = {l->late, l->defer, l->fchain, l->bchain, l->fs, l->ah, l->q_per2_ride, l->q_head_chain, l->q_head_pf,
                         l->q_head_launches, (int64_t)l->variant, (l->timeout_flag && *l->timeout_flag) ? 1 : 0};
  for (int i = 0; i < 12; ++i) out[i] = v[i];
  return DRA_OK;
}

DRA_API int dra_dqn_learner_lane_stats(dra_dqn_learner* l, int64_t* out) {
  if (!l || !out) return DRA_EINVAL;
  for (int i = 0; i < 12; ++i) out[i] = l->fs_stat[i];
  return DRA_OK;
}

static int stage_acquire(dra_dqn_learner* l, int* k_out) {
  const int k = l->stage_k;
  l->stage_k = (k + 1) % 8;
  if (l->stage_used[k]) {
    HostTimeScope waited(l->host_wait_s);
    DRA_HIP(hipEventSynchronize(l->stage_ev[k]));
    if ((l->variant & DRA_VAR_GATHER_ON_UPDATE) && l->stage_used[(k + 1) % 8]) DRA_HIP(hipEventSynchronize(l->stage_ev[(k + 1) % 8]));
  }
  l->stage_used[k] = true;
  *k_out = k;
  return DRA_OK;
}

DRA_API int dra_dqn_learner_act(dra_dqn_learner* l, const dra_dqn_step_params* prm, int use_graph, void* stream) {
  if (!l || !prm || prm->n_env < 1 || prm->n_env > kMaxEnvSteps) return DRA_EINVAL;
// ... 226 lines not shown
```

### deeprl_amd/csrc/oneshot.h

```cpp
#pragma once
#include "igemm.h"

__device__ __forceinline__ int mfma_row(int r, int h) { return (r & 3) + 8 * (r >> 2) + 4 * h; }

__device__ __forceinline__ f32x16 zero16() {
  f32x16 a;
#pragma unroll
  for (int r = 0; r < 16; ++r) a[r] = 0.f;
  return a;
}

__device__ __forceinline__ void reduce4(float* __restrict__ red, const f32x16& acc, int wave, int lane, float out[4]) {
#pragma unroll
  for (int r = 0; r < 16; ++r) red[(wave * 16 + r) * 64 + lane] = acc[r];
  __syncthreads();
#pragma unroll
  for (int q = 0; q < 4; ++q) {
    const int r = wave * 4 + q;
    out[q] = (red[(0 * 16 + r) * 64 + lane] + red[(1 * 16 + r) * 64 + lane]) +
             (red[(2 * 16 + r) * 64 + lane] + red[(3 * 16 + r) * 64 + lane]);
  }
}

struct NoRole {
// ... 187 lines not shown
        reinterpret_cast<float4*>(grad)[begin4 + i] = r;
        sq = r.x * r.x + r.y * r.y + r.z * r.z + r.w * r.w;
      }
    }
    const double d = wave_sum((double)sq);
    if (tid == 0) partials[bid] = d;
  }
};

template <int O>
struct LinDgradOne {
  static constexpr int KW = O / 4, NJ = KW / 2, LDA = O + 1, RA = 32 * O / 256;
  static constexpr int LDS_FLOATS = 32 * LDA > 4096 ? 32 * LDA : 4096;
  static_assert(O % 8 == 0 && (32 * O) % 256 == 0, "reduction split over 4 waves x 2 half-waves");
  const float* dy;
  const float* w;
  const float* xact;
  float* dx;
  int B, I, act, tiles_n;
  ChainHook hook;
  __device__ __forceinline__ void run(int bid, float* __restrict__ lds, int = 0) const { run_<false>(bid, lds); }
  template <bool COUT, bool CIN = false>
  __device__ __forceinline__ void run_(int bid, float* __restrict__ lds) const {
    const int tid = threadIdx.x, wave = tid >> 6, lane = tid & 63, li = lane & 31, h = lane >> 5;
    const int bm = bid / tiles_n, bn = bid - bm * tiles_n;
    const int m0 = bm * 32, n0 = bn * 32;
    const int ncol = min(n0 + li, I - 1);
    DRA_STAMP(TR_FC_B, 0);
    const int kb = wave * KW + h * NJ;
    float breg[NJ];
    {
      const float* wp = w + (int64_t)kb * I + ncol;
#pragma unroll
      for (int j = 0; j < NJ; ++j) breg[j] = wp[(int64_t)j * I];
    }
    float araw[RA];
    if constexpr (!CIN) {
#pragma unroll
      for (int q = 0; q < RA; ++q) {
        const int e = tid + 256 * q, row = e / O, col = e - row * O;
        araw[q] = dy[(int64_t)min(m0 + row, B - 1) * O + col];
      }
    }
    float aux[4];
    {
      const float* src = xact ? xact : dx;
#pragma unroll
      for (int q = 0; q < 4; ++q) {
        const int m = min(m0 + mfma_row(wave * 4 + q, h), B - 1);
        aux[q] = src[(int64_t)m * I + ncol];
      }
    }
    __builtin_amdgcn_sched_barrier(0);
    if constexpr (CIN) {
      mega_wait(hook.sync(0));
#pragma unroll
      for (int q = 0; q < RA; ++q) {
        const int e = tid + 256 * q, row = e / O, col = e - row * O;
        araw[q] = mega_ld<true>(dy + (int64_t)min(m0 + row, B - 1) * O + col);
      }
    }
#pragma unroll
    for (int q = 0; q < RA; ++q) {
      const int e = tid + 256 * q, row = e / O, col = e - row * O;
      lds[row * LDA + col] = araw[q];
    }
    DRA_STAMP(TR_FC_B, 1);
    __syncthreads();
    DRA_STAMP(TR_FC_B, 2);
    f32x16 acc = zero16();
    const float* ap = lds + li * LDA + kb;
#pragma unroll
    for (int j = 0; j < NJ; ++j) acc = __builtin_amdgcn_mfma_f32_32x32x2f32(ap[j], breg[j], acc, 0, 0, 0);
    DRA_STAMP(TR_FC_B, 3);
    __syncthreads();
    DRA_STAMP(TR_FC_B, 4);
    float s[4];
    reduce4(lds, acc, wave, lane, s);
#pragma unroll
    for (int q = 0; q < 4; ++q) {
      const int m = m0 + mfma_row(wave * 4 + q, h);
      if (m < B && n0 + li < I) mega_st<COUT>(&dx[(int64_t)m * I + n0 + li], xact ? s[q] * act_grad(aux[q], act) : s[q]);
    }
    DRA_STAMP(TR_FC_B, 5);
    if constexpr (COUT) mega_publish(hook.sync(0));
    DRA_STAMP_END(TR_FC_B);
  }
};

template <int I, int KS, int NT = 1>
struct LinFwdSlabsOne {
  static constexpr int KPS = I / KS, KW = KPS / 4, NJ = KW / 2, LD = KPS + 1;
  static constexpr int V = KPS / 4, NVX = 32 * V, NVW = 32 * NT * V, RX = (NVX + 255) / 256, RWV = (NVW + 255) / 256;
  static constexpr int LDS_FLOATS = (1 + NT) * 32 * LD > NT * 4096 ? (1 + NT) * 32 * LD : NT * 4096;
  static_assert(I % KS == 0 && KPS % 8 == 0, "K split: float4 rows, even k per half-wave");
  static_assert(LDS_FLOATS * 4 <= 160 * 1024, "LDS per workgroup");
  const float* x[kMaxZ];
  const float* w[kMaxZ];
  float* slabs;
  int B, O, tiles_n, tiles_m;
  const float* bias[kMaxZ] = {};
  float* out[kMaxZ] = {};
  int xcd = 0, n_groups = 0;
  __device__ __forceinline__ void run(int bid_, float* __restrict__ lds, int first = 0) const {
    const int tid = threadIdx.x, wave = tid >> 6, lane = tid & 63, li = lane & 31, h = lane >> 5;
    const int bid = xcd ? xcd_order(bid_, first, n_groups, tiles_n) : bid_;
    const int bn = bid % tiles_n;
    int r = bid / tiles_n;
    const int bm = r % tiles_m;
    r /= tiles_m;
    const int s = r % KS, z = r / KS;
    const int m0 = bm * 32, n0 = bn * 32 * NT, k0 = s * KPS;
    const float* __restrict__ xz = x[z];
    const float* __restrict__ wz = w[z];
    DRA_STAMP(TR_FC4_F, 0);
    float bias_r[NT];
#pragma unroll
    for (int t = 0; t < NT; ++t) bias_r[t] = (KS == 1 && out[z]) ? bias[z][min(n0 + 32 * t + li, O - 1)] : 0.f;
// ... 287 lines not shown
```

### deeprl_amd/csrc/oneshot_lin.h

```cpp
#pragma once
#include "oneshot.h"

typedef float lin_f4 __attribute__((ext_vector_type(4)));

template <class G, int PT = 1>
struct ConvDgradLin {
  static constexpr int S = G::S, KP = (G::KH + S - 1) / S, NPH = S * S, HP = (G::H + S - 1) / S, PP = HP * HP;
  static constexpr int OH = G::OH, P = G::P;
  static constexpr int TPP = (PP + 31) / 32, TGP = (TPP + PT - 1) / PT;
  static constexpr int OCW = G::OC / 4, OCH = OCW / 2, NT = KP * KP, NJ = NT * OCH;
  static constexpr int MT = G::C / 32;
  static constexpr int NSRC = G::OC * P;
  static constexpr int ZERO = ((OCH - 1) * P + 1 + 3) & ~3;
  static constexpr int IMG = NSRC + ZERO;
  static constexpr int RED = PT * 4096;
  static constexpr int LDS_FLOATS = IMG > RED ? IMG : RED;
  static_assert(G::KH % S == 0, "every stride phase has KP x KP taps");
  static_assert(G::OC % 32 == 0 && OCH % 4 == 0 && G::C % 32 == 0, "float4 weight runs per half-wave");
  static_assert(NSRC % 4 == 0, "float4 staging");
  const float* dy;
  const float* wt;
  const float* xact;
  float* dx;
  int B, act;
// ... 276 lines not shown
    }
    __builtin_amdgcn_sched_barrier(0);
    if constexpr (CIN) {
      mega_wait(hook.sync(0));
#pragma unroll
      for (int j = 0; j < 16; ++j) areg[j] = mega_ld<true>(dy + (int64_t)min(2 * j + h, B - 1) * O + oc);
    }
#pragma unroll
    for (int j = 0; j < 16; ++j)
      if (2 * j + h >= B) areg[j] = 0.f;
    float sq = 0.f;
#pragma unroll
    for (int t = 0; t < TPW; ++t) {
      const int it = wave + 4 * t;
      const int i0 = (gi * NI + it) * 32;
      if (it < NI && i0 < I) {
        f32x16 acc = zero16();
#pragma unroll
        for (int j = 0; j < 16; ++j) acc = __builtin_amdgcn_mfma_f32_32x32x2f32(areg[j], breg[t][j], acc, 0, 0, 0);
        const int i = i0 + li;
#pragma unroll
        for (int r = 0; r < 16; ++r) {
          const int o = o0 + mfma_row(r, h);
          if (o < O && i < I) {
            dw[(int64_t)o * I + i] = acc[r];
            sq += acc[r] * acc[r];
          }
        }
      }
    }
    DRA_STAMP(TR_FC_B, 3);
    if (db && gi == 0 && wave == 0) {
      float sb = 0.f;
#pragma unroll
      for (int j = 0; j < 16; ++j) {
        const float other = __shfl_xor(areg[j], 32, 64);
        const float even = h ? other : areg[j], odd = h ? areg[j] : other;
        sb += even;
        sb += odd;
      }
      if (h == 0 && o0 + li < O) {
        db[o0 + li] = sb;
        sq += sb * sb;
      }
    }
    if (partials) {
      const double d = wave_sum((double)sq);
      double* dl = reinterpret_cast<double*>(lds);
      if (lane == 0) dl[wave] = d;
      __syncthreads();
      if (tid == 0) partials[bid] = (dl[0] + dl[1]) + (dl[2] + dl[3]);
    }
    DRA_STAMP(TR_FC_B, 5);
  }
};

template <class G, int MTG, int SHARES, int SPI>
struct ConvWgradPers {
  using L = ConvWgradLin<G, MTG>;
  static constexpr int S = G::S, OH = G::OH, P = G::P, H = G::H, HW = G::HW;
  static constexpr int NJ = L::NJ, NGRP = L::NGRP, NTL = L::NTL, TILES = L::TILES, TPW = L::TPW, IMGF = L::IMGF, NSRC = L::NSRC;
  static constexpr bool ODD = L::ODD;
  static constexpr int BUF = (IMGF + NSRC + 4 + 3) & ~3;
  static constexpr int RED = 4 * G::OC;
  static constexpr int LDS_FLOATS = SPI * BUF + RED;
  const float* dy;
  const void* x;
  float* dw;
  float* db;
  int64_t slab_stride;
  int B;
  __host__ __device__ static int spw(int batch) { return (batch + SHARES - 1) / SHARES; }
  __host__ static int n_slabs(int batch) { return (batch + spw(batch) - 1) / spw(batch); }
  __host__ int blocks() const { return n_slabs(B) * NGRP; }
  static constexpr int pos_off(int p) { return (p / OH) * S * H + (p % OH) * S; }
  __device__ __forceinline__ void run(int bid, float* __restrict__ lds, int = 0) const {
    const int tid = threadIdx.x, wave = tid >> 6, lane = tid & 63, li = lane & 31, h = lane >> 5;
    const int per = spw(B);
    const int grp = bid % NGRP, share = bid / NGRP;
    const int b0 = share * per, b1 = min(B, b0 + per);
    const int k0 = grp * MTG * 32;
    const int c_lo = k0 / G::KK;
    const int c_hi = min((k0 + MTG * 32 - 1) / G::KK, G::C - 1);
    const int nch = c_hi - c_lo + 1;
    constexpr int NVD = NSRC / 4, RD = (NVD + 255) / 256;
    constexpr int RI = (IMGF / 4 + 255) / 256;
    const int64_t xlast4 = ((int64_t)B * G::C * HW >> 2) - 1;
    lin_f4 draw[SPI][RD], iraw[SPI][RI];
    int shift_nxt[SPI], nvi_nxt[SPI], shift[SPI];
    auto fetch = [&](int bi0) {
#pragma unroll
      for (int u = 0; u < SPI; ++u) {
        const int bi = min(bi0 + u, b1 - 1);
        const lin_f4* dyb4 = reinterpret_cast<const lin_f4*>(dy + (int64_t)bi * NSRC);
#pragma unroll
        for (int q = 0; q < RD; ++q) draw[u][q] = dyb4[min(tid + 256 * q, NVD - 1)];
        const int64_t xstart = ((int64_t)bi * G::C + c_lo) * HW;
        shift_nxt[u] = (int)(xstart & 3);
        nvi_nxt[u] = (nch * HW + shift_nxt[u] + 3) >> 2;
        const lin_f4* x4 = reinterpret_cast<const lin_f4*>(x) + (xstart >> 2);
#pragma unroll
        for (int q = 0; q < RI; ++q) {
          const int64_t f = min((int64_t)(tid + 256 * q), (int64_t)nvi_nxt[u] - 1);
          iraw[u][q] = x4[min(f, xlast4 - (xstart >> 2))];
        }
      }
// ... 89 lines not shown
```

### deeprl_amd/learner.py

```python
import ctypes
import os

import numpy as np
import torch

from . import ops
from ._lib import DraError, lib
from .optim import FlatParams
from .replay import draw_uniform_indices
from .support import Config

_ORDER = ["body.conv1.weight", "body.conv1.bias", "body.conv2.weight", "body.conv2.bias", "body.conv3.weight",
          "body.conv3.bias", "body.fc4.weight", "body.fc4.bias", "fc_head.weight", "fc_head.bias"]


_PARTITIONED_STREAMS = {}


class DqnConfig(ctypes.Structure):
    _fields_ = [("batch", ctypes.c_int32), ("n_actions", ctypes.c_int32), ("double_q", ctypes.c_int32),
                ("ksplit", ctypes.c_int32), ("centered", ctypes.c_int32), ("env_done_period", ctypes.c_int32),
                ("gamma_n", ctypes.c_float), ("gradient_clip", ctypes.c_float), ("lr", ctypes.c_float),
                ("alpha", ctypes.c_float), ("eps", ctypes.c_float), ("replay_eps", ctypes.c_float),
                ("replay_alpha", ctypes.c_float), ("variant", ctypes.c_int32), ("u8_coef", ctypes.c_double),
# ... 55 lines not shown
        cfg.batch, cfg.n_actions, cfg.double_q, cfg.ksplit, cfg.centered = batch, n_actions, int(double_q), ksplit, int(centered)
        cfg.gamma_n, cfg.gradient_clip, cfg.lr, cfg.alpha, cfg.eps = gamma_n, gradient_clip or 0.0, lr, alpha, eps
        cfg.replay_eps, cfg.replay_alpha, cfg.u8_coef = replay_eps, replay_alpha, u8_coef
        cfg.env_seed, cfg.env_done_period = env_seed, env_done_period
        cfg.head_kind, cfg.n_atoms, cfg.v_min, cfg.v_max = self.head_kind, int(n_atoms), float(v_min), float(v_max)
        cfg.optimizer, cfg.beta1, cfg.beta2 = int(optimizer), float(betas[0]), float(betas[1])
        cfg.variant = int(variant)
        cfg.n_params = self.flat.numel
        cfg.conv_end = self.flat.offsets[6]
        cfg.ring_capacity = ring.capacity
        for i, o in enumerate(self.flat.offsets):
            cfg.offset[i] = o
        self.cfg = cfg
        self.batch, self.n_actions = batch, n_actions
        h = ctypes.c_void_p()
        lib.dra_dqn_learner_create(ctypes.byref(h), ring.h, ctypes.byref(cfg), ctypes.c_void_p(self.flat.flat.data_ptr()),
                                   ctypes.c_void_p(self.target_flat.flat.data_ptr()),
                                   ctypes.c_void_p(self.flat.grad.data_ptr()), ctypes.c_void_p(self.state1.data_ptr()),
                                   ctypes.c_void_p(self.state2.data_ptr()))
        self.h = h
        ps = [ctypes.c_void_p() for _ in range(8)]
        lib.dra_dqn_learner_buffers(h, *[ctypes.byref(p) for p in ps])
        w = ops._wrap_device_pointer
        self.idx = w(ps[0].value, batch, torch.int64)
        self.sampling_prob = w(ps[1].value, batch + 1, torch.float32)
        self._loss_per = w(ps[2].value, 1, torch.float32)
        self.norm = w(ps[3].value, 1, torch.float32)
        self.n_out = n_actions * (int(n_atoms) if self.head_kind != HEAD_VANILLA else 1)
        self.q = w(ps[4].value, batch * self.n_out, torch.float32)
        self.q = self.q.view(batch, n_actions) if self.head_kind == HEAD_VANILLA else self.q.view(batch, n_actions, int(n_atoms))
        self.delta = w(ps[5].value, batch, torch.float32)
        self.prio = w(ps[6].value, batch, torch.float32)
        self.actor_q = w(ps[7].value, n_actions, torch.float32)
        self.update_cus = self.actor_cus = None
        if self.variant & ops.VAR_CU_PARTITION:
            try:
                self.stream, self.actor_stream = self._partitioned_streams()
            except DraError as e:
                import warnings
                warnings.warn("CU-partitioned streams unavailable (%s); using plain streams" % (e,))
                self.stream, self.actor_stream = torch.cuda.Stream(), torch.cuda.Stream()
                self.update_cus = self.actor_cus = None
        else:
            self.stream = torch.cuda.Stream()
            self.actor_stream = torch.cuda.Stream()
        if self.actor_cus:
            lib.dra_dqn_learner_set_actor_cus(self.h, int(self.actor_cus))
        self.ahead_stream = None
        if self.variant & ops.VAR_TARGET_AHEAD:
            self.ahead_stream = self._ahead_stream()
            lib.dra_dqn_learner_set_ahead_stream(self.h, self._sp(self.ahead_stream))
            if not self.ahead_stats()["active"]:
                self.ahead_stream = None
        self.params = StepParams()
        self._idx_view = np.ctypeslib.as_array(self.params.idx)[:batch]
        self._k = 0

    def _partitioned_streams(self):
        import os
        n_cu = torch.cuda.get_device_properties(Config.DEVICE).multi_processor_count
        n_act = max(8, min(n_cu - 8, int(os.environ.get("DRA_ACTOR_CUS", str(n_cu // 8)))))
        key = (Config.DEVICE.index, n_act)
        self.update_cus, self.actor_cus = n_cu - n_act, n_act
        if key in _PARTITIONED_STREAMS:
            return _PARTITIONED_STREAMS[key]
        actor_bits = set(range(n_act))
        words = (n_cu + 31) // 32
        out = []
        with torch.cuda.device(Config.DEVICE):
            for bits in (set(range(n_cu)) - actor_bits, actor_bits):
                mask = (ctypes.c_uint32 * words)()
                for b in bits:
                    mask[b // 32] |= 1 << (b % 32)
                h = ctypes.c_void_p()
                lib.dra_stream_create_masked(ctypes.byref(h), mask, words)
                out.append(torch.cuda.ExternalStream(h.value, device=Config.DEVICE))
        _PARTITIONED_STREAMS[key] = out
        return out

    def _ahead_stream(self):
        if not self.update_cus:
            return torch.cuda.Stream()
        key = (Config.DEVICE.index, self.actor_cus, "ahead")
        if key not in _PARTITIONED_STREAMS:
            n_cu = self.update_cus + self.actor_cus
            words = (n_cu + 31) // 32
            mask = (ctypes.c_uint32 * words)()
            for b in range(self.actor_cus, n_cu):
                mask[b // 32] |= 1 << (b % 32)
            h = ctypes.c_void_p()
            with torch.cuda.device(Config.DEVICE):
                lib.dra_stream_create_masked(ctypes.byref(h), mask, words)
            _PARTITIONED_STREAMS[key] = torch.cuda.ExternalStream(h.value, device=Config.DEVICE)
        return _PARTITIONED_STREAMS[key]

    def stage_next_indices(self, idx_next):
        a = np.ascontiguousarray(idx_next, dtype=np.int64)
        lib.dra_dqn_learner_stage_next_indices(self.h, a.ctypes.data_as(ctypes.c_void_p), int(a.size))

    def ahead_stats(self):
        out = (ctypes.c_int64 * 8)()
        lib.dra_dqn_learner_ahead_stats(self.h, out)
        return {"from_stash": int(out[0]), "in_line": int(out[1]), "skipped_slot_hazard": int(out[2]),
                "index_mismatch": int(out[3]), "active": bool(out[4])}

    def close(self):
        if self.h:
            lib.dra_dqn_learner_destroy(self.h)
            self.h = None

    def __del__(self):
        try:
            self.close()
        except Exception:
            pass

    def _sp(self, stream=None):
        return ctypes.c_void_p((stream or self.stream).cuda_stream)

    @property
    def loss(self):
        if self.head_kind == HEAD_QUANTILE:
            return self._loss_per[0]
        if self.head_kind != HEAD_VANILLA:
            return self.delta.mean()
        return self.delta.pow(2).mul(0.5).mean()

    def upload_indices(self, idx):
        idx = np.ascontiguousarray(idx, dtype=np.int64)
        lib.dra_dqn_learner_upload_indices(self.h, idx.ctypes.data_as(ctypes.c_void_p), int(idx.shape[0]), self._sp())

    def upload_sampling_prob(self, prob, beta):
        prob = np.ascontiguousarray(prob, dtype=np.float64)
        lib.dra_dqn_learner_upload_sampling_prob(self.h, prob.ctypes.data_as(ctypes.c_void_p), int(prob.shape[0]), float(beta),
                                                 self._sp())

# ... 82 lines not shown
        lib.dra_dqn_learner_keep_minibatch(self.h, int(bool(keep)))

    def sync_target(self):
        lib.dra_dqn_learner_sync_target(self.h, self._sp())

    def q_host(self, state):
        state = np.ascontiguousarray(state, dtype=np.uint8)
        if state.size != 4 * 7056:
            raise DraError("q_host: expected a uint8 [4,84,84] observation, got shape %s" % (state.shape,))
        q = np.empty(self.n_actions, dtype=np.float32)
        lib.dra_dqn_learner_q_host(self.h, state.ctypes.data_as(ctypes.c_void_p), q.ctypes.data_as(ctypes.c_void_p),
                                   self._sp())
        return q

    def profile(self):
        n = lib.dra_dqn_learner_kernel_count.raw()
        out = (ctypes.c_float * (n + 1))()
        lib.dra_dqn_learner_profile(self.h, out, n + 1, self._sp())
        names = []
        for k in range(n):
            buf = ctypes.create_string_buffer(32)
            lib.dra_dqn_learner_kernel_name(k, buf, 32)
            names.append(buf.value.decode())
        res = dict(zip(names, [float(v) for v in out[:n]]))
        res["_event_bracket"] = float(out[n])
        return res

    def kernel_replay(self, name, reps=64):
        n = lib.dra_dqn_learner_kernel_count.raw()
        for k in range(n):
            buf = ctypes.create_string_buffer(32)
            lib.dra_dqn_learner_kernel_name(k, buf, 32)
            if buf.value.decode() == name:
                out = (ctypes.c_float * 2)()
                lib.dra_dqn_learner_kernel_replay(self.h, k, int(reps), out, self._sp())
                return float(out[0]), float(out[1])
        raise DraError("kernel_replay: no kernel group named %r" % (name,))

    def chain_replay(self, which, reps=64):
        out = (ctypes.c_float * 2)()
        lib.dra_dqn_learner_chain_replay(self.h, {"fwd": 0, "bwd": 1}[which], int(reps), out, self._sp())
        return float(out[0]), float(out[1])

    CHAIN_COUNTER_CLASSES = ("fwd_conv1_to_conv2", "fwd_conv2_to_conv3", "bwd_conv3_dgrad", "bwd_conv2_dgrad", "bwd_conv3_wgrad",
                             "bwd_conv2_wgrad", "bwd_fc4_dgrad")

    def chain_set_epoch(self, epoch):
        out = (ctypes.c_int64 * 8)()
        lib.dra_dqn_learner_chain_set_epoch(self.h, int(epoch), out, 8, self._sp())
        res = {k: int(out[i]) for i, k in enumerate(self.CHAIN_COUNTER_CLASSES) if out[i]}
        res["target_ahead"] = bool(out[7])
        return res

    def synchronize(self):
        lib.dra_dqn_learner_flush(self.h, self._sp())
        self.stream.synchronize()
        self.actor_stream.synchronize()

    def host_stats(self, reset=True):
        out = (ctypes.c_double * 3)()
        lib.dra_dqn_learner_host_stats(self.h, out, int(reset))
        n = max(1.0, out[0])
        return {"calls": int(out[0]), "call_us": 1e6 * out[1] / n, "blocked_on_gpu_us": 1e6 * out[2] / n}

    def lane_stats(self):
        out = (ctypes.c_int64 * 12)()
        lib.dra_dqn_learner_lane_stats(self.h, out)
        n = max(1, int(out[0]))
        return {"steps": int(out[0]), "entries": int(out[1]), "hazard_bumps": int(out[2]), "host_waits": int(out[3]),
                "host_us_per_step": {"pacing_wait": out[4] / n / 1e3, "index_staging": out[5] / n / 1e3,
                                     "update_launches": out[6] / n / 1e3, "actor_launch": out[7] / n / 1e3,
                                     "whole_call": out[8] / n / 1e3}}

    def path_flags(self):
        out = (ctypes.c_int64 * 12)()
        lib.dra_dqn_learner_path_flags(self.h, out)
        keys = ("late", "defer", "fchain", "bchain", "fs", "ah", "per2_ride", "head_chain", "head_pf")
        res = {k: bool(out[i]) for i, k in enumerate(keys)}
        res["head_launches"], res["variant"], res["timed_out"] = int(out[9]), int(out[10]), bool(out[11])
        return res

    def invalidate_actor_copy(self):
        lib.dra_dqn_learner_invalidate_actor_copy(self.h)

    def export_state(self):
        self.synchronize()
        torch.cuda.synchronize()
        names = _param_order(self.head_kind)
        net_p = dict(self.network.named_parameters())

        def per_tensor(buf):
            out = {}
            for k in names:
                p = net_p[k]
                o = self.flat.offset_of(p)
                v = buf[o:o + p.numel()]
                if p.dim() == 4 and not p.is_contiguous():
                    oc, c, kh, kw = p.shape
                    v = v.view(c, kh, kw, oc).permute(3, 0, 1, 2)
                else:
                    v = v.view(p.shape)
                out[k] = v.detach().cpu().contiguous().clone()
            return out

        return {"params": per_tensor(self.flat.flat), "target": per_tensor(self.target_flat.flat),
                "square_avg": per_tensor(self.state1), "grad_avg": per_tensor(self.state2),
                "state1": per_tensor(self.state1), "state2": per_tensor(self.state2)}

    def _resume_buffers(self):
        n = lib.dra_dqn_learner_resume_buffer_count.raw()
        out = []
        for i in range(n):
            p, nb = ctypes.c_void_p(), ctypes.c_int64()
            name = ctypes.create_string_buffer(32)
            lib.dra_dqn_learner_resume_buffer(self.h, i, ctypes.byref(p), ctypes.byref(nb), name, 32)
            if p.value and nb.value:
                out.append((name.value.decode(), ops._wrap_device_pointer(p.value, nb.value, torch.uint8)))
        return out

    def resume_state(self):
        self.synchronize()
        torch.cuda.synchronize()
# ... 575 lines not shown
```

### deeprl_amd/ops.py

```python
import ctypes

import numpy as np
import torch

from ._lib import DraError, lib, ptr, ptr_array, stream_ptr

ACT = {None: 0, "none": 0, "relu": 1, "tanh": 2}
_f32 = torch.float32


def _dev(t):
    if not t.is_cuda:
        raise DraError("deeprl_amd ops need device tensors (got %s); there is no CPU fallback" % t.device)
    return t


def _c(t, dtype=None):
    _dev(t)
    if dtype is not None and t.dtype != dtype:
        raise DraError("expected dtype %s, got %s" % (dtype, t.dtype))
    return t if t.is_contiguous() else t.contiguous()


class Ring:
# ... 393 lines not shown
    batch = xs[0].shape[0]
    is_u8 = xs[0].dtype == torch.uint8
    xs = [_c(x, torch.uint8 if is_u8 else _f32) for x in xs]
    wts = [_c(w, _f32) for w in wts]
    bs = [_c(b, _f32) for b in bs]
    ys = [torch.empty(conv_out_shape(layer, batch), dtype=_f32, device=xs[0].device) for _ in range(nz)]
    lib.dra_conv_fwd_koc(layer, nz, ptr_array(xs), ptr_array(wts), ptr_array(bs), ptr_array(ys), batch, int(is_u8),
                         float(u8_coef if is_u8 else 1.0), ACT[act], stream_ptr())
    return ys


def conv_bwd_w_koc(layer, dy, x, ksplit=16, u8_coef=None):
    c, h, oc, k, s = _CONV_GEOM[layer]
    kk = c * k * k
    is_u8 = x.dtype == torch.uint8
    stride = (oc * kk + oc + 3) // 4 * 4
    slabs = torch.empty(ksplit * stride, dtype=_f32, device=x.device)
    lib.dra_conv_bwd_w_koc(layer, ptr(_c(dy, _f32)), ptr(_c(x)), ptr(slabs), ctypes.c_void_p(slabs.data_ptr() + 4 * oc * kk),
                           stride, ksplit, x.shape[0], int(is_u8), float(u8_coef if is_u8 else 1.0), stream_ptr())
    v = slabs.view(ksplit, stride)
    return v[:, :oc * kk], v[:, oc * kk:oc * kk + oc]


def conv_bwd_x_koc(layer, dy, wt, xact=None, act="relu"):
    c, h, oc, k, s = _CONV_GEOM[layer]
    batch = dy.shape[0]
    dx = torch.empty((batch, c, h, h), dtype=_f32, device=dy.device)
    lib.dra_conv_bwd_x_koc(layer, ptr(_c(dy, _f32)), ptr(_c(wt, _f32)), ptr(None if xact is None else _c(xact, _f32)),
                           ptr(dx), batch, ACT[act], stream_ptr())
    return dx


VAR_FUSED_BWD, VAR_ONESHOT_DGRAD, VAR_ONESHOT_FWD, VAR_ONESHOT_WGRAD = 1, 2, 4, 8
VAR_PINNED_IDX, VAR_ACTOR_V2, VAR_ACTOR_PARAMS, VAR_PIPE_GATHER, VAR_CU_PARTITION, VAR_ACTOR_V3 = 16, 32, 64, 128, 256, 512
VAR_ACTOR_FUSED_HEAD = 1024
VAR_GATHER_IN_GRAPH = 2048
VAR_ACTOR_RING = 4096
VAR_ACTOR_FUSED_CONV1 = 8192
VAR_GATHER_ON_UPDATE = 16384
VAR_RING_DIRECT = 32768
VAR_IDX_PREFETCH = 131072
VAR_DGRAD_SCATTER = 262144
VAR_LATE_FOLD = 524288
VAR_ACTOR_MEGA = 1048576
VAR_DEFER_FC4 = 8388608
VAR_ACTOR_PERSIST = 16777216
VAR_FWD_CHAIN = 33554432
VAR_BWD_CHAIN = 67108864
VAR_FLAG_SYNC = 134217728
VAR_LANE_EAGER = 268435456
VAR_TARGET_AHEAD = 536870912
VAR_BWD_CHAIN_FC = 1073741824
VAR_HEAD_CHAIN = 65536
VAR_ALL = 2097151 | 8388608 | 16777216 | 33554432 | 67108864 | 134217728 | 268435456 | 536870912 | 1073741824 | 65536


def set_tuning(mask):
    lib.dra_set_tuning(int(mask))


def get_tuning():
    m = ctypes.c_int(0)
    lib.dra_get_tuning(ctypes.byref(m))
    return m.value


def conv_wgrad_slabs(layer, batch, ksplit, variant):
    n = ctypes.c_int(0)
    lib.dra_conv_wgrad_slabs(int(layer), int(batch), int(ksplit), int(variant), ctypes.byref(n))
    return n.value


def conv_bwd_fused(layer, dy, x, wt=None, xact=None, ksplit=16, u8_coef=None, act="relu", variant=0):
    c, h, oc, k, s = _CONV_GEOM[layer]
    kk = c * k * k
    batch = x.shape[0]
    is_u8 = x.dtype == torch.uint8
    stride = (oc * kk + oc + 3) // 4 * 4
    n_slabs = conv_wgrad_slabs(layer, batch, ksplit, variant)
    slabs = torch.full((n_slabs * stride,), float("nan"), dtype=_f32, device=x.device)
    dx = torch.full((batch, c, h, h), float("nan"), dtype=_f32, device=x.device) if layer > 1 else None
    lib.dra_conv_bwd_fused(layer, ptr(_c(dy, _f32)), ptr(_c(x)), ptr(None if wt is None else _c(wt, _f32)),
                           ptr(None if xact is None else _c(xact, _f32)), ptr(slabs),
                           ctypes.c_void_p(slabs.data_ptr() + 4 * oc * kk), stride, ksplit, ptr(dx), batch, int(is_u8),
                           float(u8_coef if is_u8 else 1.0), ACT[act], int(variant), stream_ptr())
    v = slabs.view(n_slabs, stride)
    return v[:, :oc * kk], v[:, oc * kk:oc * kk + oc], dx, slabs


def conv_bwd_fused_koc(layer, dy, x, wt, ksplit=16, u8_coef=None, variant=0, xact=None):
    c, h, oc, k, s = _CONV_GEOM[layer]
    kk = c * k * k
    batch = x.shape[0]
    is_u8 = x.dtype == torch.uint8
    stride = (oc * kk + oc + 3) // 4 * 4
    n_slabs = conv_wgrad_slabs(layer, batch, ksplit, variant)
    slabs = torch.empty(n_slabs * stride, dtype=_f32, device=x.device)
    if stride != oc * kk + oc:
        slabs.view(n_slabs, stride)[:, oc * kk + oc:].zero_()
    dx = torch.empty((batch, c, h, h), dtype=_f32, device=x.device) if layer > 1 else None
    lib.dra_conv_bwd_fused(layer, ptr(_c(dy, _f32)), ptr(_c(x)), ptr(_c(wt, _f32)), ptr(None if xact is None else _c(xact, _f32)),
                           ptr(slabs), ctypes.c_void_p(slabs.data_ptr() + 4 * oc * kk), stride, ksplit, ptr(dx), batch, int(is_u8),
                           float(u8_coef if is_u8 else 1.0), ACT["relu"], int(variant), stream_ptr())
    return dx, slabs, n_slabs, stride


def fc_bwd_fused(dq, h4, dh4, x3, w4, act="relu", variant=0):
# ... 710 lines not shown
```

### include/deeprl_amd.h

```cpp
#ifndef DEEPRL_AMD_H
#define DEEPRL_AMD_H
#include <stdint.h>
#ifdef __cplusplus
extern "C" {
#endif

#define DRA_ACT_NONE 0
#define DRA_ACT_RELU 1
#define DRA_ACT_TANH 2
#define DRA_MAX_Z 4

typedef struct dra_ring dra_ring;
int dra_ring_create(dra_ring** out, int64_t capacity, int64_t frame_bytes, int64_t action_bytes, int history,
                    int n_step, double discount);
int dra_ring_shape(dra_ring* ring, int* history, int* n_step);
int dra_ring_discount(dra_ring* ring, double* discount);
int dra_ring_destroy(dra_ring* ring);
int dra_ring_pointers(dra_ring* ring, void** frames, void** actions, void** rewards, void** masks);
int dra_ring_put(dra_ring* ring, int64_t slot0, int64_t count, const void* frame_src, const void* action_src,
                 int64_t action_val, const double* reward_src, double reward_val, const int32_t* mask_src,
                 int32_t mask_val, void* stream);
int dra_ring_put_rows(dra_ring* ring, const int64_t* slot0_dev, int64_t slot0, int count, const void* frame_src,
                      int64_t frame_stride, const int64_t* action_src, const double* reward_src, const int32_t* mask_src,
                      void* stream);
// ... 137 lines not shown
int dra_noisy_linear_fwd(const float* x, const float* w_mu, const float* w_sigma, const float* b_mu, const float* b_sigma,
                         const float* noise_in, const float* noise_out_weight, const float* noise_out_bias, float* y, int rows,
                         int in_features, int out_features, int act, float* workspace, int64_t workspace_floats, void* stream);
int dra_noisy_linear_fwd_rows(const float* x, const float* w_mu, const float* w_sigma, const float* b_mu, const float* b_sigma,
                              const float* noise_in, const float* noise_out_weight, const float* noise_out_bias,
                              int64_t noise_stride, float* y, int rows, int in_features, int out_features, int act, void* stream);
int dra_rainbow_act_rows(const float* value, const float* advantage, const float* atoms, int rows, int n_actions, int n_atoms,
                         int64_t* action, float* q, void* stream);
int dra_noisy_linear_bwd(const float* g, const float* x, const float* w_mu, const float* w_sigma, const float* noise_in,
                         const float* noise_out_weight, const float* noise_out_bias, const float* x_relu, const float* dx_add,
                         float* dw_mu, float* dw_sigma, float* db_mu, float* db_sigma, float* dx, int rows, int in_features,
                         int out_features, float* workspace, int64_t workspace_floats, void* stream);
int dra_dueling_atoms_fwd(const float* value, const float* advantage, int batch, int n_actions, int n_atoms, float* logits,
                          void* stream);
int dra_dueling_atoms_bwd(const float* g_logits, int batch, int n_actions, int n_atoms, float* d_value, float* d_advantage,
                          void* stream);
int dra_per_weights_dev(const float* loss_vec, const float* sampling_prob, int batch, const float* beta_dev, float replay_eps,
                        float replay_alpha, float* out_prio, float* out_weights, void* stream);

int dra_resize_area_tab(int ssize, int dsize, int* si, float* alpha, int* offs, int max_entries);
int dra_atari_preprocess(const uint8_t* raw, int n_env, int height, int width, int out_h, int out_w, const int* x_si,
                         const float* x_alpha, const int* x_off, const int* y_si, const float* y_alpha, const int* y_off,
                         uint8_t* out, void* stream);

#define DRA_VAR_FUSED_BWD 1
#define DRA_VAR_ONESHOT_DGRAD 2
#define DRA_VAR_ONESHOT_FWD 4
#define DRA_VAR_ONESHOT_WGRAD 8
#define DRA_VAR_PINNED_IDX 16
#define DRA_VAR_ACTOR_V2 32
#define DRA_VAR_ACTOR_PARAMS 64
#define DRA_VAR_ACTOR_V3 512
#define DRA_VAR_ACTOR_FUSED_HEAD 1024
#define DRA_VAR_GATHER_IN_GRAPH 2048
#define DRA_VAR_ACTOR_RING 4096
#define DRA_VAR_ACTOR_FUSED_CONV1 8192
#define DRA_VAR_GATHER_ON_UPDATE 16384
#define DRA_VAR_RING_DIRECT 32768
#define DRA_VAR_IDX_PREFETCH 131072
#define DRA_VAR_DGRAD_SCATTER 262144
#define DRA_VAR_LATE_FOLD 524288
#define DRA_VAR_ACTOR_MEGA 1048576
#define DRA_VAR_MEASURE_DGRAD_ONLY 2097152
#define DRA_VAR_MEASURE_WGRAD_ONLY 4194304
#define DRA_VAR_DEFER_FC4 8388608
#define DRA_VAR_ACTOR_PERSIST 16777216
#define DRA_VAR_FWD_CHAIN 33554432
#define DRA_VAR_BWD_CHAIN 67108864
#define DRA_VAR_FLAG_SYNC 134217728
#define DRA_VAR_LANE_EAGER 268435456
#define DRA_VAR_TARGET_AHEAD 536870912
#define DRA_VAR_BWD_CHAIN_FC 1073741824
#define DRA_VAR_HEAD_CHAIN 65536
#define DRA_VAR_CU_PARTITION 256
#define DRA_VAR_PIPE_GATHER 128
int dra_set_tuning(int mask);
int dra_get_tuning(int* mask);
int dra_conv_wgrad_slabs(int layer, int batch, int ksplit, int variant, int* n_slabs);
int dra_conv_bwd_fused(int layer, const float* dy, const void* x, const float* wt, const float* xact, float* dw,
                       float* db, int64_t slab_stride, int ksplit, float* dx, int batch, int x_is_u8, double u8_coef,
                       int act, int variant, void* stream);
int dra_fc_bwd_fused(const float* dq, const float* h4, const float* dh4, const float* x3, const float* w4, float* dwh,
                     float* dbh, float* dw4, float* db4, float* dx3, int batch, int n_actions, int in_features, int act,
                     int variant, void* stream);
int dra_linear_fwd_slabs_one(int nz, const float* const* x, const float* const* w, int batch, int in_features,
                             int out_features, int ksplit, float* slabs, void* stream);

int dra_norm_partials(void);
int dra_grad_sqnorm(float* grad, int64_t n, const float* slabs, int n_slabs, int64_t slab_stride, double* partials,
                    void* stream);
#define DRA_MAX_FOLD_SEGS 4
typedef struct dra_fold_seg {
  int64_t begin, count;
  const float* slabs;
  int64_t slab_stride;
  int32_t n_slabs, reserved;
} dra_fold_seg;
int dra_norm_partials_max(void);
int dra_grad_sqnorm_segs(float* grad, int64_t n, const dra_fold_seg* segs, int n_segs, double* partials,
                         int* n_partials, void* stream);
int dra_grad_sqnorm_segs_blocks(int64_t n, const dra_fold_seg* segs, int n_segs, int* blocks);
int dra_clip_step_late_blocks(const dra_fold_seg* seg, int* fold_blocks);
int dra_clip_step_late(float* param, float* grad, float* state1, float* state2, int64_t n, const dra_fold_seg* seg,
                       double* partials, int n_prior, int* timeout_flag, int optimizer, float max_norm, const float* hyper,
                       int centered, const int64_t* step_dev, float* out_norm, float* param_copy, void* stream);
int dra_rmsprop_step(float* param, const float* grad, float* square_avg, float* grad_avg, int64_t n,
                     const double* partials, int n_partials, float max_norm, float lr, float alpha, float eps,
                     int centered, float* out_norm, void* stream);
int dra_rmsprop_step_copy(float* param, const float* grad, float* square_avg, float* grad_avg, int64_t n,
                          const double* partials, int n_partials, float max_norm, float lr, float alpha, float eps,
                          int centered, float* out_norm, float* param_copy, void* stream);
int dra_adam_step(float* param, const float* grad, float* exp_avg, float* exp_avg_sq, int64_t n,
                  const double* partials, int n_partials, float max_norm, float lr, float beta1, float beta2, float eps,
                  int64_t step, float* out_norm, void* stream);
int dra_adam_hyper(float lr, float beta1, float beta2, int64_t step, float* out2);
int dra_adam_step_dev(float* param, const float* grad, float* exp_avg, float* exp_avg_sq, int64_t n,
                      const double* partials, int n_partials, float max_norm, float beta1, float beta2, float eps,
                      const float* hyper_dev, float* out_norm, void* stream);
int dra_adam_step_counter(float* param, const float* grad, float* exp_avg, float* exp_avg_sq, int64_t n,
                          const double* partials, int n_partials, float max_norm, float lr, float beta1, float beta2,
                          float eps, const int64_t* step_dev, float* out_norm, float* param_copy, void* stream);
int dra_copy_f32(float* dst, const float* src, int64_t n, void* stream);
typedef struct dra_optim_lane {
  float* param;
  const float* grad;
  float* square_avg;
// ... 92 lines not shown
} dra_dqn_step_params;
typedef struct dra_dqn_learner dra_dqn_learner;
int dra_dqn_learner_create(dra_dqn_learner** out, dra_ring* ring, const dra_dqn_config* cfg, float* params,
                           float* target, float* grad, float* state1, float* state2);
int dra_dqn_learner_destroy(dra_dqn_learner* learner);
int dra_dqn_learner_buffers(dra_dqn_learner* learner, void** idx, void** sampling_prob, void** loss, void** norm,
                            void** q, void** delta, void** prio, void** actor_q);
int dra_dqn_learner_update(dra_dqn_learner* learner, int use_graph, int per, float beta, void* stream);
int dra_dqn_learner_set_per(dra_dqn_learner* learner, int per, float beta);
int dra_dqn_learner_upload_sampling_prob(dra_dqn_learner* learner, const double* prob_host, int n, float beta, void* stream);
int dra_dqn_learner_upload_indices(dra_dqn_learner* learner, const int64_t* idx_host, int n, void* stream);
int dra_dqn_learner_keep_minibatch(dra_dqn_learner* learner, int keep);
int dra_dqn_learner_wait_loss(dra_dqn_learner* learner, void* stream);
int dra_dqn_learner_profile(dra_dqn_learner* learner, float* out_ms, int n_out, void* stream);
int dra_dqn_learner_set_actor_cus(dra_dqn_learner* learner, int n_cus);
int dra_dqn_learner_flush(dra_dqn_learner* learner, void* stream);
int dra_fc4_rider_test(float* p, const float* g, float* s1, float* s2, float* p_copy, int64_t begin4, int64_t count4,
                       const float* coef, const int* pending, float lr, float alpha, float eps, int centered, int write_through,
                       void* stream);
int dra_dqn_learner_kernel_replay(dra_dqn_learner* learner, int kernel, int reps, float* out_us, void* stream);
int dra_dqn_learner_chain_replay(dra_dqn_learner* learner, int which, int reps, float* out_us, void* stream);
int dra_dqn_learner_chain_set_epoch(dra_dqn_learner* learner, uint64_t epoch, int64_t* arrivals, int n_arrivals, void* stream);
int dra_dqn_learner_last_minibatch(dra_dqn_learner* learner, void** state, void** next_state, void** action, void** reward,
                                   void** mask);
int dra_dqn_learner_kernel_name(int k, char* out, int n);
int dra_dqn_learner_kernel_count(void);
int dra_dqn_learner_sync_target(dra_dqn_learner* learner, void* stream);
int dra_dqn_learner_invalidate_actor_copy(dra_dqn_learner* learner);
int dra_dqn_learner_act(dra_dqn_learner* learner, const dra_dqn_step_params* prm, int use_graph, void* stream);
int dra_dqn_learner_q_host(dra_dqn_learner* learner, const uint8_t* state_host, float* q_host, void* stream);
int dra_dqn_learner_set_per_chain2(dra_dqn_learner* l, dra_sumtree* tree, double* stat_dev, dra_per_chain2_io* io0,
                                   dra_per_chain2_io* io1, dra_per_chain2_io* io2, dra_per_chain2_io* io3,
                                   const uint32_t* rng_words_pinned);
int dra_dqn_learner_per_chain2_seed(dra_dqn_learner* l, const int64_t* tree_idx, const int64_t* data_idx, const double* prob,
                                    float beta, uint64_t rng_cursor, uint64_t seq, void* stream);
int dra_dqn_learner_per_chain2_wait(dra_dqn_learner* l, int slot, uint64_t seq, int64_t timeout_us);
int dra_dqn_learner_step_update(dra_dqn_learner* learner, const dra_dqn_step_params* prm, void* stream_update, void* stream_actor);
int dra_dqn_learner_step_actor(dra_dqn_learner* learner, const dra_dqn_step_params* prm, void* stream_update, void* stream_actor);
int dra_dqn_learner_next_slot(dra_dqn_learner* l, int* slot);
int dra_dqn_learner_sync_loss(dra_dqn_learner* l);
int dra_dqn_learner_update_async(dra_dqn_learner* l, int use_graph, int per, float beta, void* stream_update);
int dra_dqn_learner_q_host_async(dra_dqn_learner* l, const uint8_t* state_host, float* q_host, void* stream_actor,
                                 void* stream_update);
int dra_dqn_learner_resume_buffer_count(void);
int dra_dqn_learner_resume_buffer(dra_dqn_learner* l, int index, void** ptr, int64_t* bytes, char* name, int name_len);
int dra_dqn_learner_resume_counters(dra_dqn_learner* l, int64_t* io, int n, int restore);
int dra_dqn_learner_actor_ring_push(dra_dqn_learner* learner, const dra_dqn_step_params* blocks, int n, void* stream);
int dra_dqn_learner_step(dra_dqn_learner* learner, const dra_dqn_step_params* prm, int do_update, void* stream_update,
                         void* stream_actor);

int dra_dqn_learner_host_stats(dra_dqn_learner* learner, double* out, int reset);

int dra_dqn_learner_set_ahead_stream(dra_dqn_learner* learner, void* stream);
int dra_dqn_learner_stage_next_indices(dra_dqn_learner* learner, const int64_t* idx_next, int n);
int dra_dqn_learner_ahead_stats(dra_dqn_learner* learner, int64_t* out);
int dra_dqn_learner_lane_stats(dra_dqn_learner* learner, int64_t* out);
int dra_dqn_learner_path_flags(dra_dqn_learner* learner, int64_t* out);

int dra_stream_create_masked(void** out_stream, const uint32_t* cu_mask, int n_words);
int dra_stream_destroy(void* stream);
int dra_probe_hw_id(uint32_t* out, int n_workgroups, void* stream);

int dra_dqn_learner_trace(dra_dqn_learner* learner, int n_steps);
int dra_dqn_learner_trace_read(dra_dqn_learner* learner, float* out_ms, int max_steps, int* n_steps);

#define DRA_COMM_ID_BYTES 256
typedef struct dra_comm dra_comm;
int dra_comm_unique_id(void* id_bytes);
int dra_comm_init_rank(dra_comm** out, int n_ranks, int rank, const void* id_bytes);
int dra_comm_destroy(dra_comm* comm);
int dra_comm_info(dra_comm* comm, int* n_ranks, int* rank);
int dra_allreduce_grads(float* flat_grad, int64_t count, float scale, dra_comm* comm, void* stream);
int dra_allreduce_f64(double* values, int count, dra_comm* comm, void* stream);

int dra_rms_normalize(const double* x, int n, int d, double* mean, double* var, double* count, int update, double epsilon,
                      double clip, float* out_f32, double* out_f64, void* stream);
int dra_gauss_sample(const float* mean, const float* scale, int n, int a_dim, uint64_t noise_seed, int64_t* step_dev,
                     int64_t n_global, int64_t env0, float* out_action, void* stream);
int dra_cont_env_step(double* state, int64_t* counter, const int64_t* seed, const float* action, int n, int s_dim, int a_dim,
                      int64_t horizon, double* out_reward, int32_t* out_done, void* stream);
typedef struct dra_ppo_mlp_net {
  float* param;
  float* exp_avg;
  float* exp_avg_sq;
  int64_t* step_dev;
  int32_t off_w1, off_b1, off_w2, off_b2, off_w3, off_b3, off_std, reserved;
  float lr, beta1, beta2, eps;
} dra_ppo_mlp_net;
typedef struct dra_ppo_mlp_cfg {
  int32_t state_dim, action_dim, hidden, mini_batch;
  float ratio_clip, entropy_weight;
  double kl_limit;
} dra_ppo_mlp_cfg;
int dra_ppo_mlp_supported(int state_dim, int action_dim, int hidden1, int hidden2, int mini_batch);
int dra_ppo_mlp_packed_floats(int n, int epochs, int mini_batch, int s_dim, int64_t* floats);
int dra_ppo_mlp_pack(const float* state, const float* action, const float* log_pi_a, const float* advantage, const float* ret,
                     const int64_t* perm, int n, int epochs, int mini_batch, int s_dim, int a_dim, float* out_packed, void* stream);
#define DRA_PPO_MLP_DBG_FLOATS 65536
int dra_ppo_mlp_update(const dra_ppo_mlp_cfg* cfg, const dra_ppo_mlp_net* actor, const dra_ppo_mlp_net* critic,
                       const float* packed, int n, int epochs, float* out3, int64_t* out_counts, float* dbg, void* stream);
int dra_ppo_mlp_update_profile(const dra_ppo_mlp_cfg* cfg, const dra_ppo_mlp_net* actor, const dra_ppo_mlp_net* critic,
                               const float* packed, int n, int epochs, float* out3, int64_t* out_counts, int64_t* cycles,
                               void* stream);
typedef struct dra_ppo_mlp_rollout_io {
  double* env_state;
  int64_t* env_counter;
// ... 484 lines not shown
```

Before: 11460 updates/s.

## Run FC backward on a twin stream gated by device counters alongside conv backward

Adds an opt-in twin-stream mode. The Q head kernel runs on the main stream, and the FC dgrad/wgrad kernel runs on a separate CU-partitioned stream. Spin-wait gate kernels and a retired counter order the two streams, and the conv backward chain waits on the FC dgrad done counter instead of a fused head+FC launch. The goal is to overlap FC weight gradients with conv backward. It also vectorises the dy load into LDS in the one-shot linear path with float4 reads. The twin mode costs extra launches, spin-waiting blocks and more complex synchronisation, with timeout risks.

After: 11070 updates/s. 3.4% lower.

```diff
diff --git a/deeprl_amd/csrc/actor_env.h b/deeprl_amd/csrc/actor_env.h
--- a/deeprl_amd/csrc/actor_env.h
+++ b/deeprl_amd/csrc/actor_env.h
@@ -170,10 +170,16 @@
   const int64_t* head_action;
   int head_group;
 };
+struct DraBwdChainTwin {
+  unsigned f_target;
+  const unsigned long long* retired;
+  unsigned long long retired_need;
+};
+int dra_bwd_chain_f_counter(void);
 int dra_conv_bwd_chain(const float* dy3, const float* y2, const float* wt3, float* dw3, float* db3, int64_t stride3, float* dy2,
                        const float* y1, const float* wt2, float* dw2, float* db2, int64_t stride2, float* dy1, const void* frames,
                        const int64_t* idx, float* dw1, float* db1, int64_t stride1, int batch, double u8_coef, int act,
                        const dra_fold_seg* fold3, const dra_fold_seg* fold2, float* grad, double* partials3, int* n_partials3,
                        double* partials2, int* n_partials2, double* reset_slots, int n_reset, unsigned* counters,
-                       const unsigned* epoch, int* timeout_flag, const DraBwdChainFc* fc, void* stream);
+                       const unsigned* epoch, int* timeout_flag, const DraBwdChainFc* fc, const DraBwdChainTwin* twin, void* stream);
 int dra_bwd_chain_level(int batch, int fc_in_features, unsigned epoch, unsigned* image, unsigned* arrivals);
diff --git a/deeprl_amd/csrc/fused.hip b/deeprl_amd/csrc/fused.hip
--- a/deeprl_amd/csrc/fused.hip
+++ b/deeprl_amd/csrc/fused.hip
@@ -327,12 +327,15 @@
 
 static bool fc_wgrad_one(int batch) { return batch <= 32; }
 constexpr int kFcWgradNI = 8;
-struct BwdChainN { int fd, fw, fh, d3, w3, d2, w2, w1, f3, f2; };
+struct BwdChainN {
+  int fd, fw, fh, d3, w3, d2, w2, w1, f3, f2;
+  const unsigned long long* retired; unsigned long long retired_need; int* timeout_flag;
+};
 using BD3 = ConvDgradLin<G3, 1>;
 using BD2 = ConvDgradLin<G2, 2>;
 using FCD = LinDgradOne<512>;
 using FCW = LinWgradOne<8>;
-template <bool FC>
+template <bool FC, bool F3 = FC>
 __global__ void __launch_bounds__(256) __attribute__((amdgpu_waves_per_eu(1, 2)))
 bwd_chain_kernel(const FCD fd, const FCW fw, const HeadWgradRole fh, const BD3 d3, const WG3l w3, const BD2 d2, const WG2l w2,
                  const WG1u w1, const FoldRole f3, const FoldRole f2, const BwdChainN n) {
@@ -346,9 +349,9 @@
     if (b < n.fh) { fh.run(b, dyn_lds, first); return; }
     b -= n.fh; first += n.fh;
   }
-  if (b < n.d3) { d3.run_<FC, true>(b, dyn_lds, first); return; }
+  if (b < n.d3) { d3.run_<F3, true>(b, dyn_lds, first); return; }
   b -= n.d3; first += n.d3;
-  if (b < n.w3) { w3.run_<FC, true>(b, dyn_lds, first); return; }
+  if (b < n.w3) { w3.run_<F3, true>(b, dyn_lds, first); return; }
   b -= n.w3; first += n.w3;
   if (b < n.d2) { d2.run_<true, true>(b, dyn_lds, first); return; }
   b -= n.d2; first += n.d2;
@@ -359,12 +362,25 @@
   if (b < n.f3) { f3.run_<true>(b, dyn_lds); return; }
   b -= n.f3;
   f2.run_<true>(b, dyn_lds);
+  if constexpr (F3 && !FC) {
+    if (b == n.f2 - 1 && threadIdx.x == 0) {
+      const unsigned long long t0 = wall_clock64();
+      while (__hip_atomic_load(n.retired, __ATOMIC_ACQUIRE, __HIP_MEMORY_SCOPE_AGENT) < n.retired_need) {
+        __builtin_amdgcn_s_sleep(8);
+        if (wall_clock64() - t0 > kMegaWaitTicks) {
+          __hip_atomic_store(n.timeout_flag, 1, __ATOMIC_RELAXED, __HIP_MEMORY_SCOPE_SYSTEM);
+          break;
+        }
+      }
+    }
+  }
 }
 
 constexpr int kBwdChainCounters = (2 * 32 + 3) * kChainLine;
 int dra_bwd_chain_counters(void) { return kBwdChainCounters; }
 constexpr int kBwdChainA = 0, kBwdChainB = 32 * kChainLine, kBwdChainW3 = 64 * kChainLine, kBwdChainW2 = 65 * kChainLine,
               kBwdChainF = 66 * kChainLine;
+int dra_bwd_chain_f_counter(void) { return kBwdChainF; }
 struct BwdChainArrivals { unsigned d3, d2, w3, w2, fd; };
 static int fc_dgrad_tiles(int in_features) { return (in_features + 31) / 32; }
 static BwdChainArrivals bwd_chain_arrivals(int batch, int fc_in_features) {
@@ -392,7 +408,9 @@
                        const int64_t* idx, float* dw1, float* db1, int64_t stride1, int batch, double u8_coef, int act,
                        const dra_fold_seg* fold3, const dra_fold_seg* fold2, float* grad, double* partials3, int* n_partials3,
                        double* partials2, int* n_partials2, double* reset_slots, int n_reset, unsigned* counters,
-                       const unsigned* epoch, int* timeout_flag, const DraBwdChainFc* fc, void* stream) {
+                       const unsigned* epoch, int* timeout_flag, const DraBwdChainFc* fc, const DraBwdChainTwin* twin, void* stream) {
+  if (fc && twin) return DRA_EINVAL;
+  if (twin && (!twin->retired || batch > 32)) return DRA_EINVAL;
   if (!dy3 || !y2 || !wt3 || !dw3 || !db3 || !dy2 || !y1 || !wt2 || !dw2 || !db2 || !dy1 || !frames || !dw1 || !db1 || batch < 1 ||
       batch > 32 || !n_partials3 || !n_partials2 || !fold_ok(fold3, grad, partials3) || !fold_ok(fold2, grad, partials2) || !counters ||
       !epoch || !timeout_flag)
@@ -409,6 +427,7 @@
   FoldRole f2 = make_fold_role(fold2, grad, partials2, reset_slots, n_reset);
   BwdChainN n;
   n.fd = n.fw = n.fh = 0;
+  n.retired = twin ? twin->retired : nullptr; n.retired_need = twin ? twin->retired_need : 0ull; n.timeout_flag = timeout_flag;
   n.d3 = d3.blocks(); n.w3 = w3.blocks(); n.d2 = d2.blocks(); n.w2 = w2.blocks(); n.w1 = w1.blocks(); n.f3 = f3.blocks(); n.f2 = f2.blocks();
   *n_partials3 = n.f3; *n_partials2 = n.f2;
   unsigned *cA = counters + kBwdChainA, *cB = counters + kBwdChainB, *cW3 = counters + kBwdChainW3, *cW2 = counters + kBwdChainW2,
@@ -442,6 +461,10 @@
     d3.hook.wait = cF; d3.hook.wait_stride = 0; d3.hook.wait_target = na.fd; d3.hook.slow = 1;
     w3.hook.wait = cF; w3.hook.wait_stride = 0; w3.hook.wait_target = na.fd; w3.hook.slow = 1;
   }
+  if (twin) {
+    d3.hook.wait = cF; d3.hook.wait_stride = 0; d3.hook.wait_target = twin->f_target; d3.hook.slow = 1; d3.hook.epoch = nullptr;
+    w3.hook.wait = cF; w3.hook.wait_stride = 0; w3.hook.wait_target = twin->f_target; w3.hook.slow = 1; w3.hook.epoch = nullptr;
+  }
   d2.hook = base; d2.hook.wait = cA; d2.hook.wait_stride = kChainLine; d2.hook.wait_target = na.d3;
   d2.hook.done = cB; d2.hook.done_stride = kChainLine;
   w2.hook = base; w2.hook.wait = cA; w2.hook.wait_stride = kChainLine; w2.hook.wait_target = na.d3; w2.hook.done = cW2;
@@ -462,6 +485,8 @@
     if (bytes_fc > 64 * 1024)
       if (int rc = dra_grant_lds(lds_attr, reinterpret_cast<const void*>(&bwd_chain_kernel<true>), bytes_fc)) return rc;
     hipLaunchKernelGGL(bwd_chain_kernel<true>, dim3(grid), dim3(256), bytes_fc, dra_stream(stream), fd, fw, fh, d3, w3, d2, w2, w1, f3, f2, n);
+  } else if (twin) {
+    hipLaunchKernelGGL((bwd_chain_kernel<false, true>), dim3(grid), dim3(256), bytes, dra_stream(stream), fd, fw, fh, d3, w3, d2, w2, w1, f3, f2, n);
   } else {
     hipLaunchKernelGGL(bwd_chain_kernel<false>, dim3(grid), dim3(256), bytes, dra_stream(stream), fd, fw, fh, d3, w3, d2, w2, w1, f3, f2, n);
   }
diff --git a/deeprl_amd/csrc/learner.hip b/deeprl_amd/csrc/learner.hip
--- a/deeprl_amd/csrc/learner.hip
+++ b/deeprl_amd/csrc/learner.hip
@@ -119,6 +119,12 @@
   int only_kernel;
   int only_chain;
   unsigned* hchain_dev;
+  bool twin;
+  hipStream_t tw_stream;
+  unsigned long long* tw_dev;
+  uint64_t tw_heads, tw_dgrads, tw_updates;
+  bool tw_eager;
+  unsigned tw_f;
   bool defer;
   float* defer_dev;
   bool defer_host;
@@ -313,6 +319,7 @@
   rc |= alloc_f(&l->slabs, (int64_t)cfg->ksplit * l->slab_stride);
   if (cfg->variant >= 0) l->variant = cfg->variant;
   else rc |= dra_get_tuning(&l->variant);
+  l->twin = (l->variant & DRA_VAR_TWIN_STREAM) != 0;
   if ((l->variant & DRA_VAR_RING_DIRECT) &&
       (!(l->variant & DRA_VAR_ONESHOT_WGRAD) || !(l->variant & DRA_VAR_GATHER_ON_UPDATE) || !(l->variant & DRA_VAR_PINNED_IDX)))
     l->variant &= ~DRA_VAR_RING_DIRECT;
@@ -379,6 +386,8 @@
   rc |= (int)hipMalloc(&l->aflags, (size_t)kMaxEnvSteps * 4 * sizeof(unsigned));
   rc |= (int)hipMalloc(&l->hchain_dev, 256);
   if (!rc) rc |= (int)hipMemset(l->hchain_dev, 0, 256);
+  rc |= (int)hipMalloc(&l->tw_dev, 48 * sizeof(unsigned long long));
+  if (!rc) rc |= (int)hipMemset(l->tw_dev, 0, 48 * sizeof(unsigned long long));
   rc |= (int)hipMalloc(&l->fchain_dev, (size_t)(kFwdChainCounters + 2) * sizeof(unsigned));
   if (!rc) rc |= (int)hipMemset(l->fchain_dev, 0, (size_t)(kFwdChainCounters + 2) * sizeof(unsigned));
   l->ah = false;
@@ -516,6 +525,7 @@
   if (l->all_dev) (void)hipFree(l->all_dev);
   if (l->fchain_dev) (void)hipFree(l->fchain_dev);
   if (l->hchain_dev) (void)hipFree(l->hchain_dev);
+  if (l->tw_dev) (void)hipFree(l->tw_dev);
   for (int k = 0; k < 2; ++k) {
     void* ab[] = {l->ah_y1[k], l->ah_y2[k], l->ah_y3[k], l->ah_slabs[k], l->ah_chain[k]};
     for (void* b : ab) if (b) (void)hipFree(b);
@@ -996,6 +1006,61 @@
   b -= nd;
   if (b < nw) { rl.run_<true>(b, dyn_lds); return; }
   rh.run_<true>(b - nw, dyn_lds);
+}
+
+#ifndef DRA_EXP_TWIN_SPARES
+#define DRA_EXP_TWIN_SPARES 1
+#endif
+constexpr bool kTwinSpares = DRA_EXP_TWIN_SPARES != 0;
+template <int KS>
+__global__ void __launch_bounds__(256)
+head_twin_kernel(const HeadArgs ha, const float* __restrict__ pf_w4, unsigned long long* started) {
+  __shared__ float s_h[3][512];
+  __shared__ float s_q[3][64];
+  const int b = blockIdx.x, tid = threadIdx.x;
+  if (b >= ha.B) {
+    const int pcol = (b - ha.B) * 32;
+    float4 v[16];
+#pragma unroll
+    for (int qq = 0; qq < 16; ++qq) {
+      const int e = tid + 256 * qq, row = e >> 3, c4 = e & 7;
+      v[qq] = *reinterpret_cast<const float4*>(pf_w4 + (int64_t)row * 3136 + pcol + 4 * c4);
+    }
+#pragma unroll
+    for (int qq = 0; qq < 16; ++qq) asm volatile("" :: "v"(v[qq].x), "v"(v[qq].y), "v"(v[qq].z), "v"(v[qq].w));
+    return;
+  }
+  if (tid == 0) __hip_atomic_fetch_add(started, 1ull, __ATOMIC_RELAXED, __HIP_MEMORY_SCOPE_AGENT);
+  head_fused_body<KS, true>(ha.slabs, ha.nz, ha.B, ha.A, ha.b4_on, ha.b4_tg, ha.wh_on, ha.wh_tg, ha.bh_on, ha.bh_tg, ha.action, ha.reward,
+                            ha.mask, ha.gamma_n, ha.double_q, ha.h4_out, ha.q_on, ha.q_tg, ha.q_on2, ha.delta, ha.dq, ha.dh4, ha.opt_step,
+                            ha.rs, ha.per_w, b, s_h, s_q, ha.done);
+}
+__global__ void __launch_bounds__(256) __attribute__((amdgpu_waves_per_eu(1, 2)))
+fc_bwd_twin_kernel(const LinDgradOne<512> rd, const LinWgradOne<8> rl, const HeadWgradRole rh, const int nd, const int nw,
+                   unsigned long long* started) {
+  extern __shared__ __attribute__((aligned(16))) float dyn_lds[];
+  const int b = blockIdx.x;
+  if (b < nd) {
+    if (threadIdx.x == 0) __hip_atomic_fetch_add(started, 1ull, __ATOMIC_RELAXED, __HIP_MEMORY_SCOPE_AGENT);
+    rd.run_<true, true>(b, dyn_lds);
+  } else if (b < nd + nw) {
+    rl.run_<true>(b - nd, dyn_lds);
+  } else {
+    rh.run_<true>(b - nd - nw, dyn_lds);
+  }
+}
+__global__ void tw_mark_kernel(unsigned long long* retired, unsigned long long value) {
+  __hip_atomic_store(retired, value, __ATOMIC_RELEASE, __HIP_MEMORY_SCOPE_AGENT);
+}
+__global__ void tw_gate_kernel(const unsigned long long* count, unsigned long long need, int* timeout_flag) {
+  const unsigned long long t0 = wall_clock64();
+  while (__hip_atomic_load(count, __ATOMIC_ACQUIRE, __HIP_MEMORY_SCOPE_AGENT) < need) {
+    __builtin_amdgcn_s_sleep(4);
+    if (wall_clock64() - t0 > 4 * kMegaWaitTicks) {
+      __hip_atomic_store(timeout_flag, 1, __ATOMIC_RELAXED, __HIP_MEMORY_SCOPE_SYSTEM);
+      break;
+    }
+  }
 }
 
 __global__ void __launch_bounds__(64)
@@ -1282,6 +1347,7 @@
   const bool rd = l->rd_slot >= 0;
   const bool bchain = l->bchain && rd && !l->profiling && l->only_kernel < 0 && part == 0 && !per && !(l->per2_active && l->per2_ride);
   bool head_chain = false;
+  bool twin = false;
   void *ring_frames = nullptr, *ring_actions = nullptr, *ring_rewards = nullptr, *ring_masks = nullptr;
   int ring_h = 4, ring_n = 1;
   double ring_discount = 1.0;
@@ -1316,7 +1382,7 @@
       DraFc4Rider rdr;
       if (riding) rdr = fc4_rider(l, l->pa[l->rider_q]);
       if (l->fs_capturing) dra_conv_chain_attach_announce(l->fs_count);
-      if ((l->variant & DRA_VAR_HEAD_CHAIN) && l->hchain_dev) dra_conv_chain_attach_zero(l->hchain_dev);
+      if (((l->variant & DRA_VAR_HEAD_CHAIN) || l->twin) && l->hchain_dev) dra_conv_chain_attach_zero(l->hchain_dev);
       int rcc = dra_conv_fwd_chain(ring_frames, dev_idx ? l->per2_idx + (size_t)l->rd_slot * 1024 : l->idx_pin[l->rd_slot], l->idx,
                                    pf ? l->idx_tag_dev + (size_t)l->rd_slot * 1024 : nullptr, pf ? l->rd_seq_dev : nullptr, off,
                                    l->ah_mode ? 1 : nz,
@@ -1385,8 +1451,11 @@
     const bool pf = (l->variant & DRA_VAR_ONESHOT_DGRAD) && B % 8 == 0 && B <= 32 && dra_xcd_order_enabled();
     const float* pf_w4 = pf ? P + o[P_W4] : nullptr;
     const int hb = B + (pf ? 3136 / 32 : 0);
+    twin = l->tw_eager && l->twin && l->tw_stream && chain && bchain && !per && ks4 == kFc4SplitMid && B <= 32 && nz == 2 && l->late &&
+           part == 0 && !(l->variant & (DRA_VAR_HEAD_CHAIN | DRA_VAR_BWD_CHAIN_FC)) && (l->variant & DRA_VAR_ONESHOT_DGRAD) &&
+           l->hchain_dev && l->tw_dev && !l->profiling && l->only_kernel < 0 && l->only_chain == 0 && !(l->ah && l->ah_stream);
     l->q_head_chain = head_chain ? 1 : 0; l->q_head_pf = (!head_chain && pf) ? 1 : 0; l->q_head_launches++;
-    if (head_chain) {
+    if (head_chain || twin) {
       HeadArgs ha;
       ha.slabs = l->fc4_slabs; ha.nz = nz; ha.B = B; ha.A = A; ha.b4_on = P + o[P_B4]; ha.b4_tg = T + o[P_B4]; ha.wh_on = P + o[P_WH];
       ha.wh_tg = T + o[P_WH]; ha.bh_on = P + o[P_BH]; ha.bh_tg = T + o[P_BH]; ha.action = (const int64_t*)l->action_[l->gb];
@@ -1410,9 +1479,31 @@
       rh.hook = hk;
       if (nw + 2 * A != dra_fc_bwd_fused_sq_partials(B, A, 3136)) return DRA_EINVAL;
       constexpr size_t hbytes = (size_t)LinDgradOne<512>::LDS_FLOATS * sizeof(float);
+      if (twin) {
+        unsigned arr[5];
+        if (int rca = dra_bwd_chain_level(B, 3136, 0, nullptr, arr)) return rca;
+        if ((int)arr[4] != nd) return DRA_EINVAL;
+        rd.hook.done = l->bchain_dev + dra_bwd_chain_f_counter();
+        static DraLdsAttr tw_attr;
+        if (int rcl = dra_grant_lds(tw_attr, reinterpret_cast<const void*>(&fc_bwd_twin_kernel), hbytes)) return rcl;
+        hipLaunchKernelGGL(head_twin_kernel<kFc4SplitMid>, dim3(kTwinSpares ? hb : B), dim3(256), 0, st, ha, pf_w4, l->tw_dev);
+        DRA_LAUNCH_CHECK();
+        l->tw_heads += (uint64_t)B; l->tw_dgrads += (uint64_t)nd; l->tw_updates += 1; l->tw_f += 1u;
+        hipLaunchKernelGGL(tw_gate_kernel, dim3(1), dim3(1), 0, l->tw_stream, (const unsigned long long*)l->tw_dev,
+                           (unsigned long long)l->tw_heads, l->timeout_flag);
+        DRA_LAUNCH_CHECK();
+        hipLaunchKernelGGL(fc_bwd_twin_kernel, dim3(nd + nw + 2 * A), dim3(256), hbytes, l->tw_stream, rd, rl, rh, nd, nw, l->tw_dev + 16);
+        DRA_LAUNCH_CHECK();
+        hipLaunchKernelGGL(tw_mark_kernel, dim3(1), dim3(1), 0, l->tw_stream, l->tw_dev + 32, (unsigned long long)l->tw_updates);
+        DRA_LAUNCH_CHECK();
+        hipLaunchKernelGGL(tw_gate_kernel, dim3(1), dim3(1), 0, st, (const unsigned long long*)(l->tw_dev + 16),
+                           (unsigned long long)l->tw_dgrads, l->timeout_flag);
+        l->fs_stat[9]++;
+      } else {
       static DraLdsAttr lds_attr;
       if (int rcl = dra_grant_lds(lds_attr, reinterpret_cast<const void*>(&head_fc_bwd_kernel<kFc4SplitMid>), hbytes)) return rcl;
       hipLaunchKernelGGL(head_fc_bwd_kernel<kFc4SplitMid>, dim3(B + nd + nw + 2 * A), dim3(256), hbytes, st, ha, rd, rl, rh, nd, nw);
+      }
     } else
     if (ks4 == kFc4SplitWide)
       hipLaunchKernelGGL(head_fused_kernel<kFc4SplitWide>, dim3(hb), dim3(256), 0, st, (const float*)l->fc4_slabs, nz, B, A,
@@ -1448,7 +1539,7 @@
   float* G = l->g;
   float* S = l->slabs;
   if (l->variant & (DRA_VAR_FUSED_BWD | DRA_VAR_ONESHOT_WGRAD)) {
-    const int var = l->variant;
+    const int var = l->variant & ~DRA_VAR_TWIN_STREAM;
     const bool own = var & DRA_VAR_ONESHOT_WGRAD;
     float* dw[3]; float* dbs[3]; int64_t stride[3];
     const int wi[3] = {P_W1, P_W2, P_W3}, bi_[3] = {P_B1, P_B2, P_B3};
@@ -1462,15 +1553,17 @@
       dra_fold_seg segs[3];
       conv_fold_segs(l, segs);
       const int nfc_expect = dra_fc_bwd_fused_sq_partials(B, NO, 3136), n3_expect = (int)((l->lstride[2] / 4 + 63) / 64), n2_expect = (int)((l->lstride[1] / 4 + 63) / 64);
-      const bool fc_in_chain = bchain && (l->variant & DRA_VAR_BWD_CHAIN_FC) && B <= 32 && !head_chain;
-      int nfc = (l->only_kernel >= 0 || (l->only_chain == 2 && !fc_in_chain) || head_chain) ? nfc_expect : 0, n3 = l->only_kernel >= 0 ? n3_expect : 0, n2 = l->only_kernel >= 0 ? n2_expect : 0;
-      if (l->only_chain != 2 && !fc_in_chain && !head_chain)
+      const bool fc_in_chain = bchain && (l->variant & DRA_VAR_BWD_CHAIN_FC) && B <= 32 && !head_chain && !twin;
+      int nfc = (l->only_kernel >= 0 || (l->only_chain == 2 && !fc_in_chain) || head_chain || twin) ? nfc_expect : 0, n3 = l->only_kernel >= 0 ? n3_expect : 0, n2 = l->only_kernel >= 0 ? n2_expect : 0;
+      if (l->only_chain != 2 && !fc_in_chain && !head_chain && !twin)
       STEP(K_FC4_BX, dra_fc_bwd_fused_sq(l->dq, l->h4, l->dh4, l->y3[0], P + o[P_W4], G + o[P_WH], G + o[P_BH], G + o[P_W4],
                                          G + o[P_B4], l->dy3, B, NO, 3136, DRA_ACT_RELU, var, l->partials, &nfc,
                                          c.head_kind != DRA_HEAD_VANILLA ? l->action_[l->gb] : nullptr, c.n_atoms, s));
       if (l->profiling) DRA_HIP(hipEventRecord(l->ev[K_CONV3_BW], st));
       if (bchain) {
         DraBwdChainFc fcb;
+        DraBwdChainTwin twb;
+        if (twin) { twb.f_target = l->tw_f * (unsigned)(3136 / 32); twb.retired = l->tw_dev + 32; twb.retired_need = l->tw_updates; }
         if (fc_in_chain) {
           fcb.dq = l->dq; fcb.h4 = l->h4; fcb.dh4 = l->dh4; fcb.x3 = l->y3[0]; fcb.w4 = P + o[P_W4]; fcb.dwh = G + o[P_WH];
           fcb.dbh = G + o[P_BH]; fcb.dw4 = G + o[P_W4]; fcb.db4 = G + o[P_B4]; fcb.n_actions = NO; fcb.in_features = 3136;
@@ -1482,7 +1575,8 @@
                                      DRA_ACT_RELU, &segs[2], &segs[1], G, l->partials + nfc_expect, &n3,
                                      l->partials + nfc_expect + n3_expect, &n2,
                                      l->partials + nfc_expect + n3_expect + n2_expect, l->late_nfold, l->bchain_dev,
-                                     l->fchain_dev + kFwdChainCounters, l->timeout_flag, fc_in_chain ? &fcb : nullptr, s);
+                                     l->fchain_dev + kFwdChainCounters, l->timeout_flag, fc_in_chain ? &fcb : nullptr,
+                                     twin ? &twb : nullptr, s);
         if (rcb) return rcb;
         if (nfc != nfc_expect || n3 != n3_expect || n2 != n2_expect) return DRA_EINVAL;
         l->late_nprior = nfc + n3 + n2;
@@ -1837,6 +1931,7 @@
     }
     if (rc == DRA_OK) rc = (int)hipMemsetAsync(l->fchain_dev, 0, (size_t)(kFwdChainCounters + 1) * sizeof(unsigned), st);
     if (rc == DRA_OK) rc = (int)hipMemsetAsync(l->bchain_dev, 0, (size_t)dra_bwd_chain_counters() * sizeof(unsigned), st);
+    l->tw_f = 0;
     if (rc == DRA_OK) rc = (int)hipStreamSynchronize(st);
     g.reset();
     if (rc != DRA_OK) return rc;
@@ -1869,11 +1964,13 @@
       arrivals[7] = 1;
     }
   if (l->bchain) {
-    const bool fc = (l->variant & DRA_VAR_BWD_CHAIN_FC) != 0;
+    const bool fc = (l->variant & DRA_VAR_BWD_CHAIN_FC) != 0 || (l->twin && l->c.batch <= 32);
     std::vector<unsigned> bimg((size_t)dra_bwd_chain_counters());
     if (int rcb = dra_bwd_chain_level(l->c.batch, fc ? 3136 : 0, e, bimg.data(), ba)) return rcb;
+    l->tw_f = e;
     DRA_HIP(hipMemcpy(l->bchain_dev, bimg.data(), bimg.size() * sizeof(unsigned), hipMemcpyHostToDevice));
     for (int i = 0; i < 5; ++i) arrivals[2 + i] = ba[i];
+    if (!(l->variant & DRA_VAR_BWD_CHAIN_FC)) arrivals[6] = 0;
   }
   return DRA_OK;
 }
@@ -3053,12 +3150,14 @@
   l->fs_on = false;
   DRA_HIP(hipStreamSynchronize(su));
   DRA_HIP(hipStreamSynchronize(sa));
+  if (l->tw_stream) DRA_HIP(hipStreamSynchronize(l->tw_stream));
   if (l->ah && l->ah_stream) {
     DRA_HIP(hipStreamSynchronize(l->ah_stream));
     l->ah_valid = false;
     l->ah_next_set = false;
     DRA_HIP(hipMemsetAsync(l->fchain_dev, 0, (size_t)(kFwdChainCounters + 1) * sizeof(unsigned), su));
     DRA_HIP(hipMemsetAsync(l->bchain_dev, 0, (size_t)dra_bwd_chain_counters() * sizeof(unsigned), su));
+    l->tw_f = 0;
     DRA_HIP(hipStreamSynchronize(su));
   }
   l->last_done = nullptr;
@@ -3104,7 +3203,9 @@
   l->rd_slot = q;
   l->rider_q = l->defer ? ((q + 3) & 3) : -1;
   l->fs_capturing = true;
+  l->tw_eager = true;
   int rc = run_body(l, st, 0, 0.f, 0, 0);
+  l->tw_eager = false;
   l->fs_capturing = false;
   l->rider_q = -1;
   if (rc == DRA_OK) rc = launch_optimizer(l, st, l->pa[q], l->defer ? q : -1);
@@ -3234,6 +3335,13 @@
   return DRA_OK;
 }
 
+DRA_API int dra_dqn_learner_set_twin_stream(dra_dqn_learner* l, void* stream) {
+  if (!l) return DRA_EINVAL;
+  if (int rcl = fs_leave_any(l)) return rcl;
+  l->tw_stream = stream ? dra_stream(stream) : nullptr;
+  return DRA_OK;
+}
+
 DRA_API int dra_dqn_learner_set_ahead_stream(dra_dqn_learner* l, void* stream) {
   if (!l) return DRA_EINVAL;
   if (int rcl = fs_leave_any(l)) return rcl;
diff --git a/deeprl_amd/csrc/oneshot.h b/deeprl_amd/csrc/oneshot.h
--- a/deeprl_amd/csrc/oneshot.h
+++ b/deeprl_amd/csrc/oneshot.h
@@ -263,6 +263,22 @@
       }
     }
     __builtin_amdgcn_sched_barrier(0);
+    if constexpr (CIN && kWideLd4 && O % 4 == 0 && RA % 4 == 0) {
+      mega_wait(hook.sync(0));
+      constexpr int O4 = O / 4;
+#pragma unroll
+      for (int q = 0; q < RA / 4; ++q) {
+        const int e = tid + 256 * q, row = e / O4, c4 = e - row * O4;
+        const dra_f4 v = mega_ld4<true>(reinterpret_cast<const dra_f4*>(dy), (int64_t)min(m0 + row, B - 1) * O4 + c4);
+        araw[4 * q] = v.x; araw[4 * q + 1] = v.y; araw[4 * q + 2] = v.z; araw[4 * q + 3] = v.w;
+      }
+#pragma unroll
+      for (int q = 0; q < RA / 4; ++q) {
+        const int e = tid + 256 * q, row = e / O4, c4 = e - row * O4;
+        float* d = lds + row * LDA + 4 * c4;
+        d[0] = araw[4 * q]; d[1] = araw[4 * q + 1]; d[2] = araw[4 * q + 2]; d[3] = araw[4 * q + 3];
+      }
+    } else {
     if constexpr (CIN) {
       mega_wait(hook.sync(0));
 #pragma unroll
@@ -275,6 +291,7 @@
     for (int q = 0; q < RA; ++q) {
       const int e = tid + 256 * q, row = e / O, col = e - row * O;
       lds[row * LDA + col] = araw[q];
+    }
     }
     DRA_STAMP(TR_FC_B, 1);
     __syncthreads();
diff --git a/deeprl_amd/csrc/oneshot_lin.h b/deeprl_amd/csrc/oneshot_lin.h
--- a/deeprl_amd/csrc/oneshot_lin.h
+++ b/deeprl_amd/csrc/oneshot_lin.h
@@ -352,6 +352,7 @@
       if (tid == 0) partials[bid] = (dl[0] + dl[1]) + (dl[2] + dl[3]);
     }
     DRA_STAMP(TR_FC_B, 5);
+    DRA_STAMP_END(TR_FC_B);
   }
 };
 
diff --git a/deeprl_amd/learner.py b/deeprl_amd/learner.py
--- a/deeprl_amd/learner.py
+++ b/deeprl_amd/learner.py
@@ -131,6 +131,9 @@
             lib.dra_dqn_learner_set_ahead_stream(self.h, self._sp(self.ahead_stream))
             if not self.ahead_stats()["active"]:
                 self.ahead_stream = None
+        self.twin_stream = None
+        if self.variant & ops.VAR_TWIN_STREAM:
+            self.set_twin_stream(True)
         self.params = StepParams()
         self._idx_view = np.ctypeslib.as_array(self.params.idx)[:batch]
         self._k = 0
@@ -157,10 +160,14 @@
         _PARTITIONED_STREAMS[key] = out
         return out
 
-    def _ahead_stream(self):
+    def set_twin_stream(self, on):
+        self.twin_stream = self._ahead_stream("twin") if on else None
+        lib.dra_dqn_learner_set_twin_stream(self.h, self._sp(self.twin_stream) if on else None)
+
+    def _ahead_stream(self, name="ahead"):
         if not self.update_cus:
             return torch.cuda.Stream()
-        key = (Config.DEVICE.index, self.actor_cus, "ahead")
+        key = (Config.DEVICE.index, self.actor_cus, name)
         if key not in _PARTITIONED_STREAMS:
             n_cu = self.update_cus + self.actor_cus
             words = (n_cu + 31) // 32
@@ -349,6 +356,9 @@
         res["target_ahead"] = bool(out[7])
         return res
 
+    def flush(self):
+        lib.dra_dqn_learner_flush(self.h, self._sp())
+
     def synchronize(self):
         lib.dra_dqn_learner_flush(self.h, self._sp())
         self.stream.synchronize()
@@ -365,6 +375,7 @@
         lib.dra_dqn_learner_lane_stats(self.h, out)
         n = max(1, int(out[0]))
         return {"steps": int(out[0]), "entries": int(out[1]), "hazard_bumps": int(out[2]), "host_waits": int(out[3]),
+                "twin_updates": int(out[9]),
                 "host_us_per_step": {"pacing_wait": out[4] / n / 1e3, "index_staging": out[5] / n / 1e3,
                                      "update_launches": out[6] / n / 1e3, "actor_launch": out[7] / n / 1e3,
                                      "whole_call": out[8] / n / 1e3}}
diff --git a/deeprl_amd/ops.py b/deeprl_amd/ops.py
--- a/deeprl_amd/ops.py
+++ b/deeprl_amd/ops.py
@@ -469,7 +469,8 @@
 VAR_TARGET_AHEAD = 536870912
 VAR_BWD_CHAIN_FC = 1073741824
 VAR_HEAD_CHAIN = 65536
-VAR_ALL = 2097151 | 8388608 | 16777216 | 33554432 | 67108864 | 134217728 | 268435456 | 536870912 | 1073741824 | 65536
+VAR_TWIN_STREAM = 2097152
+VAR_ALL = 2097151 | 8388608 | 16777216 | 33554432 | 67108864 | 134217728 | 268435456 | 536870912 | 1073741824 | 65536 | 2097152
 
 
 def set_tuning(mask):
diff --git a/include/deeprl_amd.h b/include/deeprl_amd.h
--- a/include/deeprl_amd.h
+++ b/include/deeprl_amd.h
@@ -213,6 +213,7 @@
 #define DRA_VAR_TARGET_AHEAD 536870912
 #define DRA_VAR_BWD_CHAIN_FC 1073741824
 #define DRA_VAR_HEAD_CHAIN 65536
+#define DRA_VAR_TWIN_STREAM 2097152
 #define DRA_VAR_CU_PARTITION 256
 #define DRA_VAR_PIPE_GATHER 128
 int dra_set_tuning(int mask);
@@ -411,6 +412,7 @@
 int dra_dqn_learner_host_stats(dra_dqn_learner* learner, double* out, int reset);
 
 int dra_dqn_learner_set_ahead_stream(dra_dqn_learner* learner, void* stream);
+int dra_dqn_learner_set_twin_stream(dra_dqn_learner* learner, void* stream);
 int dra_dqn_learner_stage_next_indices(dra_dqn_learner* learner, const int64_t* idx_next, int n);
 int dra_dqn_learner_ahead_stats(dra_dqn_learner* learner, int64_t* out);
 int dra_dqn_learner_lane_stats(dra_dqn_learner* learner, int64_t* out);
```
